# kessel/dune-pnp

Hardware: NVIDIA B200
Metric: newton_step_dofs_per_s (higher is better)
Workload: dtype f64

## Files before the change

### dune_pnp_b200/csrc/pnp_amg.cu

```cuda
#include <cub/cub.cuh>
#include <cusolverDn.h>

#include <chrono>
#include <cmath>
#include <cstdlib>
#include <cstring>

#include "pnp_common.cuh"
#include "pnp_spmv_tma.cuh"
#include "pnp_sweep.cuh"

namespace pnp {

std::shared_ptr<SweepPlan> sweep_plan_build(Ctx&, const SweepView&, int F);
void sweep_gs(Ctx&, const SweepPlan&, const SweepView&, const double* vals, long stride, const double* d, double* x, int dir);

namespace {

constexpr int BLK = 256;

struct Level {
  int nv = 0; long nslots = 0;
  const int* rp = nullptr; const unsigned* col = nullptr; const double* vals = nullptr;
  DBuf<int> rp_own; DBuf<unsigned> col_own; DBuf<double> vals_own;
  DBuf<double> dinv, x, x2, b, r;
  double lmax = 2.0;
  DBuf<int> agg, par1;
  DBuf<int> agg_ptr, agg_mem;
  DBuf<int> seg_ptr, seg_items;
  DBuf<unsigned char> seg_w;
  double alpha = 1.0;
  Ctx* lc = nullptr;
  Vec u; Matrix Amat;
  const unsigned char* dm = nullptr;
  bool redisc = false;
  DBuf<XY> xy_own; DBuf<unsigned char> dmask_own;
  std::shared_ptr<SweepPlan> gs_plan;
};

}

struct Amg {
  int NP = 1, F = 1;
  bool symbolic = false;
  long nv0 = -1, nslots0 = -1;
  long mg_epoch = -1;
  double sym_key = 0.0;
  double omega = 0.7, alpha = 1.6;
  int coarse_sweeps = 40;
  int gamma = 1;
  int wlevels = 99;
  int smoother = 0;
  double cheb_ratio = 8.0;
  int comp0 = 0;
  int pre_steps = -1, post_steps = -1;
  int dense_max = 4096, dense_n = 0;
  cusolverDnHandle_t cus = nullptr;
  DBuf<double> dense, dense_work;
  DBuf<int> dense_piv, dense_info;
  bool distributed = false;
  bool redisc = false;
  DBuf<double> grhs;
  std::unique_ptr<Solver> rep_solver; Matrix rep_A; Vec rep_u; DBuf<double> rep_x;
  int n_geo = 0;
  std::vector<std::unique_ptr<Level>> L;
  DBuf<unsigned char> tmp;
  void* temp(size_t bytes) { if (bytes > tmp.n) tmp.alloc(bytes); return tmp.p; }
  cudaGraphExec_t cg_exec = nullptr;
  bool cg_failed = false;
  int cg_calls = 0;
  double cg_key[8] = {0, 0, 0, 0, 0, 0, 0, 0};
  std::vector<std::pair<double*, double*>> cg_before, cg_after;
  long cg_launches = 0; double cg_bytes[Ctx::ACC_N] = {0, 0, 0, 0, 0, 0};
  void cg_reset() { if (cg_exec) cudaGraphExecDestroy(cg_exec); cg_exec = nullptr; cg_calls = 0; }
  ~Amg() { if (cg_exec) cudaGraphExecDestroy(cg_exec); if (cus) cusolverDnDestroy(cus); }
};

namespace {

__device__ __forceinline__ unsigned hash32(unsigned x) {
  x ^= x >> 16; x *= 0x7feb352du; x ^= x >> 15; x *= 0x846ca68bu; x ^= x >> 16;
  return x;
}
__global__ void k_mis_select(const int* __restrict__ rp, const unsigned* __restrict__ col, int nv,
                             const unsigned char* __restrict__ st, unsigned char* __restrict__ st_out) {
  for (int v = blockIdx.x * blockDim.x + threadIdx.x; v < nv; v += gridDim.x * blockDim.x) {
    unsigned char s = st[v];
    if (s == 0) {
      const unsigned pv = hash32((unsigned)v);
      bool win = true;
      for (int k = rp[v] + 1; k < rp[v + 1]; k++) {
        const int w = (int)(col[k] & STAR_VMASK);
        if (w >= nv || w == v || st[w] != 0) continue;
        const unsigned pw = hash32((unsigned)w);
        if (pw > pv || (pw == pv && w > v)) { win = false; break; }
      }
      if (win) s = 1;
    }
    st_out[v] = s;
  }
}
__global__ void k_mis_cover(const int* __restrict__ rp, const unsigned* __restrict__ col, int nv,
                            unsigned char* __restrict__ st, int* __restrict__ undecided) {
  int local = 0;
  for (int v = blockIdx.x * blockDim.x + threadIdx.x; v < nv; v += gridDim.x * blockDim.x) {
    if (st[v] != 0) continue;
    bool covered = false;
    for (int k = rp[v] + 1; k < rp[v + 1]; k++) {
      const int w = (int)(col[k] & STAR_VMASK);
      if (w < nv && st[w] == 1) { covered = true; break; }
    }
    if (covered) st[v] = 2; else local++;
  }
  if (local) atomicAdd(undecided, local);
}
__global__ void k_root_flag(const unsigned char* __restrict__ st, int nv, int* __restrict__ flag) {
  for (int v = blockIdx.x * blockDim.x + threadIdx.x; v < nv; v += gridDim.x * blockDim.x) flag[v] = st[v] == 1;
}
__global__ void k_attach(const int* __restrict__ rp, const unsigned* __restrict__ col, const double* __restrict__ vals,
                         int nv, const unsigned char* __restrict__ st, const int* __restrict__ root_id,
                         int* __restrict__ agg) {
  for (int v = blockIdx.x * blockDim.x + threadIdx.x; v < nv; v += gridDim.x * blockDim.x) {
    if (st[v] == 1) { agg[v] = root_id[v]; continue; }
    double best = -1.0; int bw = -1;
    for (int k = rp[v] + 1; k < rp[v + 1]; k++) {
      const int w = (int)(col[k] & STAR_VMASK);
      if (w >= nv || st[w] != 1) continue;
      const double s = fabs(vals[k]);
      if (s > best || (s == best && w < bw)) { best = s; bw = w; }
    }
    agg[v] = root_id[bw];
  }
}
__global__ void k_coarse_keys(const int* __restrict__ rp, const unsigned* __restrict__ col, int nv,
                              const int* __restrict__ agg, uint64_t* __restrict__ keys, int* __restrict__ slot_id) {
  for (int v = blockIdx.x * blockDim.x + threadIdx.x; v < nv; v += gridDim.x * blockDim.x) {
    const unsigned I = (unsigned)agg[v];
    for (int k = rp[v]; k < rp[v + 1]; k++) {
      const unsigned w = col[k] & STAR_VMASK;
      if (w >= (unsigned)nv) { keys[k] = ~0ull; slot_id[k] = k; continue; }
      const unsigned J = (unsigned)agg[w];
      keys[k] = ((uint64_t)I << 32) | (J == I ? 0u : J + 1u);
      slot_id[k] = k;
    }
  }
}
__global__ void k_coarse_cols(const uint64_t* __restrict__ ukeys, long n, unsigned* __restrict__ col) {
  for (long i = blockIdx.x * (long)blockDim.x + threadIdx.x; i < n; i += (long)gridDim.x * blockDim.x) {
    const unsigned lo = (unsigned)(ukeys[i] & 0xffffffffu);
    col[i] = lo == 0 ? (unsigned)(ukeys[i] >> 32) : lo - 1u;
  }
}
__global__ void k_row_starts(const uint64_t* __restrict__ ukeys, long n, int nc, int* __restrict__ rp) {
  for (int I = blockIdx.x * blockDim.x + threadIdx.x; I <= nc; I += gridDim.x * blockDim.x)
    rp[I] = (int)lower_bound_u64(ukeys, n, (uint64_t)(unsigned)I << 32);
}
__global__ void k_lower_bounds_i32(const int* __restrict__ sorted, int n, int m, int* __restrict__ out) {
  for (int I = blockIdx.x * blockDim.x + threadIdx.x; I <= m; I += gridDim.x * blockDim.x) {
    int lo = 0, hi = n;
    while (lo < hi) { int mid = (lo + hi) >> 1; if (sorted[mid] < I) lo = mid + 1; else hi = mid; }
    out[I] = lo;
  }
}
__global__ void k_iota(int* a, int n) {
  for (int i = blockIdx.x * blockDim.x + threadIdx.x; i < n; i += gridDim.x * blockDim.x) a[i] = i;
}

template <int NP>
__global__ void k_galerkin(const int* __restrict__ seg_ptr, const int* __restrict__ seg_items,
                           const unsigned char* __restrict__ seg_w, long nsc, const double* __restrict__ vf, long nsf, double* __restrict__ vc,
                           const unsigned char* __restrict__ dmask, const unsigned* __restrict__ colf, const int* __restrict__ rpf,
                           int comp0) {
  for (long cs = blockIdx.x * (long)blockDim.x + threadIdx.x; cs < nsc; cs += (long)gridDim.x * blockDim.x) {
    double acc[NP];
#pragma unroll
    for (int p = 0; p < NP; p++) acc[p] = 0.0;
    constexpr int U = 4;
    const int t1 = seg_ptr[cs + 1];
    for (int t0 = seg_ptr[cs]; t0 < t1; t0 += U) {
      int s[U]; double w[U]; double v[U][NP];
#pragma unroll
      for (int q = 0; q < U; q++) {
        const bool ok = t0 + q < t1;
        s[q] = ok ? seg_items[t0 + q] : -1;
        const unsigned char wc = (ok && seg_w) ? seg_w[t0 + q] : 0;
        w[q] = ok ? (wc == 0 ? 1.0 : (wc == 1 ? 0.5 : 0.25)) : 0.0;
      }
#pragma unroll
      for (int q = 0; q < U; q++)
#pragma unroll
        for (int p = 0; p < NP; p++) v[q][p] = s[q] >= 0 ? vf[p * nsf + s[q]] : 0.0;
      if (dmask) {
#pragma unroll
        for (int q = 0; q < U; q++) {
          if (s[q] < 0) continue;
          const unsigned wv = colf[s[q]] & STAR_VMASK;
          const unsigned m = dmask[wv];
          if (m && rpf[wv] == s[q]) {
            if (NP == 1) { if ((m >> comp0) & 1u) v[q][0] = 0.0; }
            else if (NP == PNP_COMPACT_PLANES) { if (m & 1u) v[q][0] = 0.0; }
            else {
              if (m & 1u) v[q][0] = 0.0;
              if (m & 2u) v[q][NP == 7 ? 4 : 0] = 0.0;
              if (m & 4u) v[q][NP == 7 ? 6 : 0] = 0.0;
            }
          }
        }
      }
#pragma unroll
      for (int q = 0; q < U; q++)
        if (s[q] >= 0) {
#pragma unroll
          for (int p = 0; p < NP; p++) acc[p] += w[q] * v[q][p];
        }
    }
#pragma unroll
    for (int p = 0; p < NP; p++) vc[p * nsc + cs] = acc[p];
  }
}
template <int NP>
__global__ void k_dinv(const int* __restrict__ rp, const double* __restrict__ vals, long stride, int nv,
                       double* __restrict__ dinv) {
  for (int v = blockIdx.x * blockDim.x + threadIdx.x; v < nv; v += gridDim.x * blockDim.x) {
    const int s = rp[v];
    if (NP == 1) { const double d = vals[s]; dinv[v] = d != 0.0 ? 1.0 / d : 0.0; }
    else {
      const PnpBlock B = pnp_block_at<NP>(vals, stride, s);
      const double a = B.a, b = B.b, c_ = B.c, d = B.d, e = B.e, f = B.f, g = B.g;
      const double det = a * e * g - b * d * g - c_ * e * f;
      double* o = dinv + 9l * v;
      const double scale = fabs(a * e * g) + fabs(b * d * g) + fabs(c_ * e * f);
      if (fabs(det) > 1e-12 * scale && scale > 0.0) {
        const double id = 1.0 / det;
        o[0] = e * g * id;   o[1] = -b * g * id;           o[2] = -c_ * e * id;
        o[3] = -d * g * id;  o[4] = (a * g - c_ * f) * id; o[5] = c_ * d * id;
        o[6] = -e * f * id;  o[7] = b * f * id;            o[8] = (a * e - b * d) * id;
      } else {
        for (int i = 0; i < 9; i++) o[i] = 0.0;
        o[0] = a != 0.0 ? 1.0 / a : 0.0; o[4] = e != 0.0 ? 1.0 / e : 0.0; o[8] = g != 0.0 ? 1.0 / g : 0.0;
      }
    }
  }
}
template <int F>
__global__ void k_jacobi0(const double* __restrict__ dinv, const double* __restrict__ b, double omega,
                          double* __restrict__ x, int nv, double* __restrict__ dvec) {
  for (int v = blockIdx.x * blockDim.x + threadIdx.x; v < nv; v += gridDim.x * blockDim.x) {
    if (F == 1) {
      const double z = omega * dinv[v] * b[v];
      x[v] = z; if (dvec) dvec[v] = z;
    } else {
      const double* B = dinv + 9l * v;
      const double r0 = b[3l * v], r1 = b[3l * v + 1], r2 = b[3l * v + 2];
#pragma unroll
      for (int k = 0; k < 3; k++) {
        const double z = omega * (B[3 * k] * r0 + B[3 * k + 1] * r1 + B[3 * k + 2] * r2);
        x[3l * v + k] = z; if (dvec) dvec[3l * v + k] = z;
      }
    }
  }
}
template <int NP>
__global__ void k_gershgorin(const int* __restrict__ rp, const double* __restrict__ vals, long stride, int nv,
                             unsigned long long* __restrict__ out) {
  double best = 0.0;
  for (int v = blockIdx.x * blockDim.x + threadIdx.x; v < nv; v += gridDim.x * blockDim.x) {
    const int s0 = rp[v], s1 = rp[v + 1];
    if (NP == 1) {
      double sum = 0.0;
      for (int s = s0; s < s1; s++) sum += fabs(vals[s]);
      const double d = fabs(vals[s0]);
      if (d > 0.0) best = fmax(best, sum / d);
    } else {
      double s0_ = 0.0, s1_ = 0.0, s2_ = 0.0;
      for (int s = s0; s < s1; s++) {
        const PnpBlock B = pnp_block_at<NP>(vals, stride, s);
        s0_ += fabs(B.a) + fabs(B.b) + fabs(B.c);
        s1_ += fabs(B.d) + fabs(B.e);
        s2_ += fabs(B.f) + fabs(B.g);
      }
      const PnpBlock D = pnp_block_at<NP>(vals, stride, s0);
      const double d0 = fabs(D.a), d1 = fabs(D.e), d2 = fabs(D.g);
      if (d0 > 0.0) best = fmax(best, s0_ / d0);
      if (d1 > 0.0) best = fmax(best, s1_ / d1);
      if (d2 > 0.0) best = fmax(best, s2_ / d2);
    }
  }
  for (int o = 16; o > 0; o >>= 1) best = fmax(best, __shfl_xor_sync(0xffffffffu, best, o));
  if ((threadIdx.x & 31) == 0) atomicMax(out, (unsigned long long)__double_as_longlong(best));
}
template <int F>
__global__ void k_restrict(const int* __restrict__ agg_ptr, const int* __restrict__ agg_mem, const int* __restrict__ par1,
                           int nc, const double* __restrict__ r, double* __restrict__ bc) {
  for (int I = blockIdx.x * blockDim.x + threadIdx.x; I < nc; I += gridDim.x * blockDim.x) {
    double acc[F];
#pragma unroll
    for (int k = 0; k < F; k++) acc[k] = 0.0;
    for (int t = agg_ptr[I]; t < agg_ptr[I + 1]; t++) {
      const long v = agg_mem[t];
      const double w = (par1 && par1[v] >= 0) ? 0.5 : 1.0;
#pragma unroll
      for (int k = 0; k < F; k++) acc[k] += w * r[F * v + k];
    }
#pragma unroll
    for (int k = 0; k < F; k++) bc[(long)F * I + k] = acc[k];
  }
}
template <int F>
__global__ void k_prolong(const int* __restrict__ agg, const int* __restrict__ par1, int nv, const double* __restrict__ xc,
                          double alpha, double* __restrict__ x, const unsigned char* __restrict__ dmask, int comp0) {
  for (int v = blockIdx.x * blockDim.x + threadIdx.x; v < nv; v += gridDim.x * blockDim.x) {
    const long I = agg[v];
    const long J = par1 ? par1[v] : -1;
    const unsigned m = dmask ? (F == 3 ? dmask[v] : (dmask[v] >> comp0) & 1u) : 0u;
#pragma unroll
    for (int k = 0; k < F; k++)
      if (!((m >> k) & 1u))
        x[(long)F * v + k] += alpha * (J >= 0 ? 0.5 * (xc[F * I + k] + xc[F * J + k]) : xc[F * I + k]);
  }
}
__global__ void k_level_geometry(const int* __restrict__ int2ext_c, const int* __restrict__ ext2int_f, const XY* __restrict__ xy_f,
                                 const unsigned char* __restrict__ dmask_f, int nvc, XY* __restrict__ xy_c,
                                 unsigned char* __restrict__ dmask_c) {
  for (int i = blockIdx.x * blockDim.x + threadIdx.x; i < nvc; i += gridDim.x * blockDim.x) {
    const int j = ext2int_f[int2ext_c[i]];
    xy_c[i] = xy_f[j]; dmask_c[i] = dmask_f[j];
  }
}
__global__ void k_geo_parents(const int* __restrict__ int2ext_f, int nvf, int nvc, const uint64_t* __restrict__ edges,
                              const int* __restrict__ ext2int_c, int* __restrict__ par0, int* __restrict__ par1) {
  for (int i = blockIdx.x * blockDim.x + threadIdx.x; i < nvf; i += gridDim.x * blockDim.x) {
    const int e = int2ext_f[i];
    if (e < nvc) { par0[i] = ext2int_c[e]; par1[i] = -1; }
    else {
      const uint64_t k = edges[e - nvc];
      par0[i] = ext2int_c[(int)(k >> 32)]; par1[i] = ext2int_c[(int)(k & 0xffffffffu)];
    }
  }
}
__global__ void k_geo_pairs(const int* __restrict__ par0, const int* __restrict__ par1, int nvf, int nrows_c,
                            int* __restrict__ key, int* __restrict__ val) {
  for (int i = blockIdx.x * blockDim.x + threadIdx.x; i < nvf; i += gridDim.x * blockDim.x) {
    key[2 * i] = (par0[i] >= 0 && par0[i] < nrows_c) ? par0[i] : 0x7fffffff; val[2 * i] = i;
    key[2 * i + 1] = (par1[i] >= 0 && par1[i] < nrows_c) ? par1[i] : 0x7fffffff; val[2 * i + 1] = i;
  }
}
template <int F>
__global__ void k_inject(const int* __restrict__ par0, const int* __restrict__ par1, int nvf, const double* __restrict__ uf,
                         double* __restrict__ uc) {
  for (int i = blockIdx.x * blockDim.x + threadIdx.x; i < nvf; i += gridDim.x * blockDim.x)
    if (par1[i] < 0 && par0[i] >= 0) {
#pragma unroll
      for (int k = 0; k < F; k++) uc[(long)F * par0[i] + k] = uf[(long)F * i + k];
    }
}
template <int F>
__global__ void k_mask_dirichlet(double* __restrict__ b, const unsigned char* __restrict__ dmask, int nv, int comp0) {
  for (int v = blockIdx.x * blockDim.x + threadIdx.x; v < nv; v += gridDim.x * blockDim.x) {
    const unsigned m = F == 3 ? dmask[v] : (dmask[v] >> comp0) & 1u;
#pragma unroll
    for (int k = 0; k < F; k++) if ((m >> k) & 1u) b[(long)F * v + k] = 0.0;
  }
}
template <int NP>
__global__ void k_dense_fill_global(const int* __restrict__ rp, const unsigned* __restrict__ col, const double* __restrict__ vals,
                                    long stride, int nrows, const int* __restrict__ gid, double* __restrict__ Ad, long n,
                                    const unsigned char* __restrict__ dmask, int comp0) {
  constexpr int F = NP == 1 ? 1 : 3;
  for (int r = blockIdx.x * blockDim.x + threadIdx.x; r < nrows; r += gridDim.x * blockDim.x) {
    const long rg = gid[r];
    for (int s = rp[r]; s < rp[r + 1]; s++) {
      const long cg = gid[col[s] & STAR_VMASK];
      const unsigned dm = (dmask && s == rp[r]) ? dmask[r] : 0u;
      if (NP == 1) { if (!((dm >> comp0) & 1u)) atomicAdd(&Ad[cg * n + rg], vals[s]); }
      else {
        const PnpBlock B = pnp_block_at<NP>(vals, stride, s);
#pragma unroll
        for (int ki = 0; ki < 3; ki++)
#pragma unroll
          for (int kj = 0; kj < 3; kj++)
            if (pnp_plane(ki, kj) >= 0 && !(ki == kj && ((dm >> ki) & 1u))) atomicAdd(&Ad[(F * cg + kj) * n + F * rg + ki], B.at(ki, kj));
      }
    }
  }
}
template <int F>
__global__ void k_to_global(const double* __restrict__ loc, const int* __restrict__ gid, int nrows, double* __restrict__ glob) {
  for (int v = blockIdx.x * blockDim.x + threadIdx.x; v < nrows; v += gridDim.x * blockDim.x)
#pragma unroll
    for (int k = 0; k < F; k++) atomicAdd(&glob[(long)F * gid[v] + k], loc[(long)F * v + k]);
}
template <int F>
__global__ void k_add_from_global(const double* __restrict__ glob, const int* __restrict__ gid, int nrows, double alpha,
                                  double* __restrict__ x, const unsigned char* __restrict__ dmask, int comp0) {
  for (int v = blockIdx.x * blockDim.x + threadIdx.x; v < nrows; v += gridDim.x * blockDim.x) {
    const unsigned m = F == 3 ? dmask[v] : (dmask[v] >> comp0) & 1u;
#pragma unroll
    for (int k = 0; k < F; k++) if (!((m >> k) & 1u)) x[(long)F * v + k] += alpha * glob[(long)F * gid[v] + k];
  }
}
template <int F>
__global__ void k_from_global(const double* __restrict__ glob, const int* __restrict__ gid, int nloc, double* __restrict__ loc) {
  for (int v = blockIdx.x * blockDim.x + threadIdx.x; v < nloc; v += gridDim.x * blockDim.x)
#pragma unroll
    for (int k = 0; k < F; k++) loc[(long)F * v + k] = glob[(long)F * gid[v] + k];
}
__device__ __forceinline__ int find_slot(const int* rp, const unsigned* col, int I, int J) {
  for (int s = rp[I]; s < rp[I + 1]; s++) if ((int)(col[s] & STAR_VMASK) == J) return s;
  return -1;
}
__global__ void k_geo_items(const int* __restrict__ rpf, const unsigned* __restrict__ colf, int nvf,
                            const int* __restrict__ par0, const int* __restrict__ par1, const int* __restrict__ rpc,
                            const unsigned* __restrict__ colc, int* __restrict__ key, unsigned* __restrict__ val,
                            int* __restrict__ err) {
  for (int i = blockIdx.x * blockDim.x + threadIdx.x; i < nvf; i += gridDim.x * blockDim.x) {
    const int I[2] = {par0[i], par1[i]};
    for (int s = rpf[i]; s < rpf[i + 1]; s++) {
      const int j = (int)(colf[s] & STAR_VMASK);
      const int J[2] = {par0[j], par1[j]};
#pragma unroll
      for (int a = 0; a < 2; a++)
#pragma unroll
        for (int b = 0; b < 2; b++) {
          const long o = 4l * s + 2 * a + b;
          if (I[a] < 0 || J[b] < 0) { key[o] = 0x7fffffff; val[o] = 0; continue; }
          const int cs = find_slot(rpc, colc, I[a], J[b]);
          if (cs < 0) { atomicExch(err, 1); key[o] = 0x7fffffff; val[o] = 0; continue; }
          const unsigned wc = (I[1] >= 0 ? 1u : 0u) + (J[1] >= 0 ? 1u : 0u);
          key[o] = cs; val[o] = (unsigned)s | (wc << 29);
        }
    }
  }
}
__global__ void k_geo_unpack(const unsigned* __restrict__ val, long n, int* __restrict__ items, unsigned char* __restrict__ w) {
  for (long t = blockIdx.x * (long)blockDim.x + threadIdx.x; t < n; t += (long)gridDim.x * blockDim.x) {
    items[t] = (int)(val[t] & 0x1fffffffu); w[t] = (unsigned char)(val[t] >> 29);
  }
}

#define KL(c, kern, n, ...)                                                                              \
  do { kern<<<grid_for((n), BLK), BLK, 0, (c).stream>>>(__VA_ARGS__); PNP_CHECK_LAUNCH(); (c).launches++; } while (0)

template <int EPI>
void level_op(Ctx& c, const Amg& A, const Level& l, const double* x, const double* b, double* y, double omega_or_c2 = -1.0,
              double c1 = 0.0, double* dvec = nullptr) {
  StarOpArgs a{l.rp, l.col, l.vals, l.nslots, l.nv, x, y};
  a.b = b; a.dinv = l.dinv.p; a.block = A.F == 3; a.omega = omega_or_c2 < 0 ? A.omega : omega_or_c2; a.c1 = c1; a.dvec = dvec;
  const bool fine = &l == A.L[0].get();
  if (A.distributed) halo_exchange(*l.lc, const_cast<double*>(x), A.F);
  if (fine) c.prof_mark(EPI == EPI_RESIDUAL ? 1 : 2);
  launch_star_op_auto<EPI, 0>(c, A.NP, a, fine);
  if (fine) c.prof_mark();
}

bool coarsen(Ctx& c, Amg& A, int li) {
  Level& f = *A.L[li];
  const int nv = f.nv;
  DBuf<unsigned char> st(nv), st2(nv);
  st.zero(c.stream);
  DBuf<int> d_und(1);
  for (int round = 0; round < 200; round++) {
    KL(c, k_mis_select, nv, f.rp, f.col, nv, st.p, st2.p);
    std::swap(st.p, st2.p);
    d_und.zero(c.stream);
    KL(c, k_mis_cover, nv, f.rp, f.col, nv, st.p, d_und.p);
    int und = 0;
    d_und.download(&und, 1, c.stream);
    if (und == 0) break;
    PNP_REQUIRE(round < 199, PNP_E_ARG, "AMG: independent-set selection did not terminate");
  }
  DBuf<int> flag(nv), root_id(nv);
  KL(c, k_root_flag, nv, st.p, nv, flag.p);
  size_t bytes = 0;
  cub::DeviceScan::ExclusiveSum(nullptr, bytes, flag.p, root_id.p, nv, c.stream);
  PNP_CUDA(cub::DeviceScan::ExclusiveSum(A.temp(bytes), bytes, flag.p, root_id.p, nv, c.stream));
  int last_id = 0, last_flag = 0;
  PNP_CUDA(cudaMemcpyAsync(&last_id, root_id.p + nv - 1, sizeof(int), cudaMemcpyDeviceToHost, c.stream));
  PNP_CUDA(cudaMemcpyAsync(&last_flag, flag.p + nv - 1, sizeof(int), cudaMemcpyDeviceToHost, c.stream));
  PNP_CUDA(cudaStreamSynchronize(c.stream));
  const int nc = last_id + last_flag;
  if (nc < 1 || nc > 0.8 * nv) return false;
  f.alpha = A.alpha;
  f.agg.alloc(nv);
  KL(c, k_attach, nv, f.rp, f.col, f.vals, nv, st.p, root_id.p, f.agg.p);
  {
    DBuf<int> ids(nv), agg_sorted(nv);
    f.agg_mem.alloc(nv); f.agg_ptr.alloc(nc + 1);
    KL(c, k_iota, nv, ids.p, nv);
    cub::DeviceRadixSort::SortPairs(nullptr, bytes, f.agg.p, agg_sorted.p, ids.p, f.agg_mem.p, nv, 0, 32, c.stream);
    PNP_CUDA(cub::DeviceRadixSort::SortPairs(A.temp(bytes), bytes, f.agg.p, agg_sorted.p, ids.p, f.agg_mem.p, nv, 0, 32,
                                            c.stream));
    KL(c, k_lower_bounds_i32, nc + 1, agg_sorted.p, nv, nc, f.agg_ptr.p);
  }
  auto nl = std::make_unique<Level>();
  {
    const long ns = f.nslots;
    PNP_REQUIRE(ns < (1l << 31), PNP_E_MESH, "AMG: too many matrix slots on one level");
    DBuf<uint64_t> keys(ns), skeys(ns), ukeys(ns);
    DBuf<int> slot(ns), counts(ns + 1), d_nu(1);
    f.seg_items.alloc(ns);
    KL(c, k_coarse_keys, nv, f.rp, f.col, nv, f.agg.p, keys.p, slot.p);
    cub::DeviceRadixSort::SortPairs(nullptr, bytes, keys.p, skeys.p, slot.p, f.seg_items.p, (int)ns, 0, 64, c.stream);
    PNP_CUDA(cub::DeviceRadixSort::SortPairs(A.temp(bytes), bytes, keys.p, skeys.p, slot.p, f.seg_items.p, (int)ns, 0, 64,
                                            c.stream));
    cub::DeviceRunLengthEncode::Encode(nullptr, bytes, skeys.p, ukeys.p, counts.p, d_nu.p, (int)ns, c.stream);
    PNP_CUDA(cub::DeviceRunLengthEncode::Encode(A.temp(bytes), bytes, skeys.p, ukeys.p, counts.p, d_nu.p, (int)ns, c.stream));
    int nu = 0;
    d_nu.download(&nu, 1, c.stream);
    {
      uint64_t lastkey = 0;
      PNP_CUDA(cudaMemcpyAsync(&lastkey, ukeys.p + (nu - 1), sizeof(uint64_t), cudaMemcpyDeviceToHost, c.stream));
      PNP_CUDA(cudaStreamSynchronize(c.stream));
      if (lastkey == ~0ull) nu--;
    }
    nl->nv = nc; nl->nslots = nu;
    PNP_CUDA(cudaMemsetAsync(counts.p + nu, 0, sizeof(int), c.stream));
    f.seg_ptr.alloc((size_t)nu + 1);
    cub::DeviceScan::ExclusiveSum(nullptr, bytes, counts.p, f.seg_ptr.p, nu + 1, c.stream);
    PNP_CUDA(cub::DeviceScan::ExclusiveSum(A.temp(bytes), bytes, counts.p, f.seg_ptr.p, nu + 1, c.stream));
    nl->rp_own.alloc((size_t)nc + 1); nl->col_own.alloc(nu);
    KL(c, k_row_starts, nc + 1, ukeys.p, (long)nu, nc, nl->rp_own.p);
    KL(c, k_coarse_cols, nu, ukeys.p, (long)nu, nl->col_own.p);
    c.launches += 8;
    PNP_CUDA(cudaStreamSynchronize(c.stream));
  }
  nl->vals_own.alloc((size_t)A.NP * nl->nslots);
  nl->rp = nl->rp_own.p; nl->col = nl->col_own.p; nl->vals = nl->vals_own.p;
  A.L.push_back(std::move(nl));
  return true;
}

void coarsen_geometric(Ctx& c, Amg& A, int li, const HierLevel& h, const int* int2ext_f, bool redisc) {
  Level& f = *A.L[li];
  const int nvf = f.nv, nvc = (int)h.nv;
  size_t bytes = 0;
  f.agg.alloc(nvf); f.par1.alloc(nvf);
  KL(c, k_geo_parents, nvf, int2ext_f, nvf, nvc, h.edges.p, h.ext2int.p, f.agg.p, f.par1.p);
  {
    DBuf<int> key(2 * (size_t)nvf), val(2 * (size_t)nvf), skey(2 * (size_t)nvf), sval(2 * (size_t)nvf);
    KL(c, k_geo_pairs, nvf, f.agg.p, f.par1.p, nvf, nvc, key.p, val.p);
    cub::DeviceRadixSort::SortPairs(nullptr, bytes, key.p, skey.p, val.p, sval.p, 2 * nvf, 0, 32, c.stream);
    PNP_CUDA(cub::DeviceRadixSort::SortPairs(A.temp(bytes), bytes, key.p, skey.p, val.p, sval.p, 2 * nvf, 0, 32, c.stream));
    f.agg_ptr.alloc((size_t)nvc + 1);
    KL(c, k_lower_bounds_i32, nvc + 1, skey.p, 2 * nvf, nvc, f.agg_ptr.p);
    int nvalid = 0;
    PNP_CUDA(cudaMemcpyAsync(&nvalid, f.agg_ptr.p + nvc, sizeof(int), cudaMemcpyDeviceToHost, c.stream));
    PNP_CUDA(cudaStreamSynchronize(c.stream));
    f.agg_mem.alloc(nvalid);
    PNP_CUDA(cudaMemcpyAsync(f.agg_mem.p, sval.p, (size_t)nvalid * sizeof(int), cudaMemcpyDeviceToDevice, c.stream));
    PNP_CUDA(cudaStreamSynchronize(c.stream));
  }
  auto nl = std::make_unique<Level>();
  nl->nv = nvc; nl->nslots = h.nslots; nl->rp = h.rp.p; nl->col = h.adj.p;
  nl->redisc = redisc;
  if (redisc) {
    nl->xy_own.alloc(nvc); nl->dmask_own.alloc(nvc);
    KL(c, k_level_geometry, nvc, h.int2ext.p, c.ext2int.p, c.xy.p, c.dmask.p, nvc, nl->xy_own.p, nl->dmask_own.p);
    nl->dm = nl->dmask_own.p;
    nl->u.fields = A.F; nl->u.d.alloc((size_t)A.F * nvc);
  } else {
    const long n4 = 4 * f.nslots;
    PNP_REQUIRE(n4 < (1l << 31) && f.nslots < (1l << 29), PNP_E_MESH, "multigrid: too many matrix slots on one level");
    DBuf<int> key(n4), skey(n4), err(1);
    DBuf<unsigned> val(n4), sval(n4);
    err.zero(c.stream);
    KL(c, k_geo_items, nvf, f.rp, f.col, nvf, f.agg.p, f.par1.p, nl->rp, nl->col, key.p, val.p, err.p);
    int herr = 0;
    err.download(&herr, 1, c.stream);
    PNP_REQUIRE(herr == 0, PNP_E_MESH, "multigrid: refinement levels are not nested");
    cub::DeviceRadixSort::SortPairs(nullptr, bytes, key.p, skey.p, val.p, sval.p, (int)n4, 0, 32, c.stream);
    PNP_CUDA(cub::DeviceRadixSort::SortPairs(A.temp(bytes), bytes, key.p, skey.p, val.p, sval.p, (int)n4, 0, 32, c.stream));
    key.release(); val.release();
    f.seg_ptr.alloc((size_t)nl->nslots + 1);
    KL(c, k_lower_bounds_i32, nl->nslots + 1, skey.p, (int)n4, (int)nl->nslots, f.seg_ptr.p);
    int nvalid = 0;
    PNP_CUDA(cudaMemcpyAsync(&nvalid, f.seg_ptr.p + nl->nslots, sizeof(int), cudaMemcpyDeviceToHost, c.stream));
    PNP_CUDA(cudaStreamSynchronize(c.stream));
    f.seg_items.alloc(nvalid); f.seg_w.alloc(nvalid);
    KL(c, k_geo_unpack, nvalid, sval.p, (long)nvalid, f.seg_items.p, f.seg_w.p);
    PNP_CUDA(cudaStreamSynchronize(c.stream));
    c.launches += 4;
  }
  f.alpha = 1.0;
  nl->vals_own.alloc((size_t)A.NP * nl->nslots);
  nl->vals = nl->vals_own.p;
  A.L.push_back(std::move(nl));
}

void alloc_work(Ctx& c, Amg& A, Level& l) {
  const size_t n = (size_t)A.F * l.nv, nall = (A.distributed && l.lc) ? (size_t)A.F * l.lc->nv : n;
  l.dinv.alloc(A.F == 3 ? 9 * (size_t)l.nv : n); l.x.alloc(nall); l.x2.alloc(nall); l.b.alloc(nall); l.r.alloc(nall);
  l.x.zero(c.stream); l.x2.zero(c.stream); l.b.zero(c.stream); l.r.zero(c.stream);
}

void coarsen_distributed(Ctx& c, Amg& A, int li, MgLevelRef& ref) {
  Level& f = *A.L[li];
  Ctx& fc = *f.lc; Ctx& kc = *ref.lc;
  const int nvf_all = (int)fc.nv, nvc = (int)kc.n_own;
  size_t bytes = 0;
  f.agg.alloc(nvf_all); f.par1.alloc(nvf_all);
  PNP_CUDA(cudaMemcpyAsync(f.agg.p, ref.par0.p, nvf_all * sizeof(int), cudaMemcpyDeviceToDevice, c.stream));
  PNP_CUDA(cudaMemcpyAsync(f.par1.p, ref.par1.p, nvf_all * sizeof(int), cudaMemcpyDeviceToDevice, c.stream));
  {
    DBuf<int> key(2 * (size_t)nvf_all), val(2 * (size_t)nvf_all), skey(2 * (size_t)nvf_all), sval(2 * (size_t)nvf_all);
    KL(c, k_geo_pairs, nvf_all, f.agg.p, f.par1.p, nvf_all, nvc, key.p, val.p);
    cub::DeviceRadixSort::SortPairs(nullptr, bytes, key.p, skey.p, val.p, sval.p, 2 * nvf_all, 0, 32, c.stream);
    PNP_CUDA(cub::DeviceRadixSort::SortPairs(A.temp(bytes), bytes, key.p, skey.p, val.p, sval.p, 2 * nvf_all, 0, 32, c.stream));
    f.agg_ptr.alloc((size_t)nvc + 1);
    KL(c, k_lower_bounds_i32, nvc + 1, skey.p, 2 * nvf_all, nvc, f.agg_ptr.p);
    int nvalid = 0;
    PNP_CUDA(cudaMemcpyAsync(&nvalid, f.agg_ptr.p + nvc, sizeof(int), cudaMemcpyDeviceToHost, c.stream));
    PNP_CUDA(cudaStreamSynchronize(c.stream));
    f.agg_mem.alloc(nvalid);
    PNP_CUDA(cudaMemcpyAsync(f.agg_mem.p, sval.p, (size_t)nvalid * sizeof(int), cudaMemcpyDeviceToDevice, c.stream));
    PNP_CUDA(cudaStreamSynchronize(c.stream));
  }
  f.alpha = 1.0;
  auto nl = std::make_unique<Level>();
  nl->lc = &kc; nl->nv = nvc; nl->nslots = kc.nslots; nl->rp = kc.rp.p; nl->col = kc.adj.p;
  nl->dm = kc.dmask.p;
  nl->u.fields = A.F; nl->u.d.alloc((size_t)A.F * kc.nv); nl->u.d.zero(c.stream);
  nl->Amat.op = A.F == 3 ? OP_PNP : OP_PB; nl->Amat.nplanes = A.NP;
  nl->Amat.vals.alloc((size_t)A.NP * kc.nslots);
  nl->vals = nl->Amat.vals.p;
  A.L.push_back(std::move(nl));
}

void dense_factor(Ctx& c, Amg& A);

void dense_factor_global(Ctx& c, Amg& A);
void replica_setup(Ctx& c, Amg& A);

const double* level_values(Ctx& c, Amg& A, int li, const double* uf, int comp0) {
  Level& l = *A.L[li]; Level& n = *A.L[li + 1];
  if (n.redisc) {
    if (A.F == 1) KL(c, k_inject<1>, l.nv, l.agg.p, l.par1.p, l.nv, uf, n.u.d.p);
    else KL(c, k_inject<3>, l.nv, l.agg.p, l.par1.p, l.nv, uf, n.u.d.p);
    c.acct(Ctx::ACC_TRANSFER, 8.0 * l.nv + 16.0 * A.F * n.nv);
    Operator op = c.last_op; op.aux0 = op.aux1 = -1;
    assemble_jacobian_on(c, StarView{n.rp, n.col, n.xy_own.p, n.dmask_own.p, n.nv}, n.nslots, op, n.u.d.p, n.vals_own.p,
                         A.NP, c.last_mode, c.last_eps);
    return n.u.d.p;
  }
  if (A.NP == 1)
    KL(c, k_galerkin<1>, n.nslots, l.seg_ptr.p, l.seg_items.p, l.seg_w.p, n.nslots, l.vals, l.nslots, n.vals_own.p, l.dm, l.col, l.rp, comp0);
  else if (A.NP == PNP_COMPACT_PLANES)
    KL(c, k_galerkin<PNP_COMPACT_PLANES>, n.nslots, l.seg_ptr.p, l.seg_items.p, l.seg_w.p, n.nslots, l.vals, l.nslots, n.vals_own.p, l.dm, l.col, l.rp, comp0);
  else
    KL(c, k_galerkin<7>, n.nslots, l.seg_ptr.p, l.seg_items.p, l.seg_w.p, n.nslots, l.vals, l.nslots, n.vals_own.p, l.dm, l.col, l.rp, comp0);
  c.acct(Ctx::ACC_ASSEMBLY, 8.0 * A.NP * ((double)l.nslots + (double)n.nslots) + 5.0 * (double)l.seg_items.n + 4.0 * (double)n.nslots);
  return nullptr;
}

void level_dinv(Ctx& c, Amg& A, Level& l) {
  if (A.NP == 1) KL(c, k_dinv<1>, l.nv, l.rp, l.vals, l.nslots, l.nv, l.dinv.p);
  else if (A.NP == PNP_COMPACT_PLANES) KL(c, k_dinv<PNP_COMPACT_PLANES>, l.nv, l.rp, l.vals, l.nslots, l.nv, l.dinv.p);
  else KL(c, k_dinv<7>, l.nv, l.rp, l.vals, l.nslots, l.nv, l.dinv.p);
}

void gershgorin_bounds(Ctx& c, Amg& A) {
  DBuf<unsigned long long> d_l(A.L.size());
  d_l.zero(c.stream);
  for (size_t li = 0; li < A.L.size(); li++) {
    Level& l = *A.L[li];
    if (A.NP == 1) KL(c, k_gershgorin<1>, l.nv, l.rp, l.vals, l.nslots, l.nv, d_l.p + li);
    else if (A.NP == PNP_COMPACT_PLANES) KL(c, k_gershgorin<PNP_COMPACT_PLANES>, l.nv, l.rp, l.vals, l.nslots, l.nv, d_l.p + li);
    else KL(c, k_gershgorin<7>, l.nv, l.rp, l.vals, l.nslots, l.nv, d_l.p + li);
  }
  if (A.distributed) allreduce_max_u64(c, d_l.p, A.L.size());
  std::vector<unsigned long long> h = d_l.to_host(c.stream);
  for (size_t li = 0; li < A.L.size(); li++) {
    double v; std::memcpy(&v, &h[li], sizeof v);
    A.L[li]->lmax = (v > 0.0 && std::isfinite(v)) ? v : 2.0;
  }
}

void numeric(Ctx& c, Amg& A, int comp0) {
  if (A.distributed) {
    PNP_REQUIRE(c.last_u, PNP_E_ARG, "distributed multigrid needs the state of the last Jacobian assembly (the vector must stay alive)");
    PNP_REQUIRE(c.last_vals == A.L[0]->vals, PNP_E_ARG,
                "distributed multigrid re-discretises its coarse levels: the matrix must be the Jacobian of the last assembly");
    const double* uf = c.last_u;
    for (size_t li = 0; li + 1 < A.L.size(); li++) {
      Level& l = *A.L[li]; Level& n = *A.L[li + 1];
      const int nvf_all = (int)l.lc->nv;
      if (A.F == 1) KL(c, k_inject<1>, nvf_all, l.agg.p, l.par1.p, nvf_all, uf, n.u.d.p);
      else KL(c, k_inject<3>, nvf_all, l.agg.p, l.par1.p, nvf_all, uf, n.u.d.p);
      c.acct(Ctx::ACC_TRANSFER, 8.0 * nvf_all + 16.0 * A.F * n.nv);
      Operator op = c.last_op; op.aux0 = op.aux1 = -1;
      n.Amat.op = op.op;
      n.lc->launches = 0;
      assemble_jacobian(*n.lc, op, n.u, n.Amat, c.last_mode, c.last_eps);
      c.absorb(*n.lc);
      uf = n.u.d.p;
    }
    for (size_t li = 0; li < A.L.size(); li++) {
      Level& l = *A.L[li];
      level_dinv(c, A, l);
      c.acct(Ctx::ACC_ASSEMBLY, (4.0 + 8.0 * A.NP + (A.F == 3 ? 72.0 : 8.0)) * l.nv);
    }
    if (c.mg_replica) replica_setup(c, A); else dense_factor_global(c, A);
    if (A.smoother == 1) gershgorin_bounds(c, A);
    return;
  }
  const double* uf = c.last_u;
  for (size_t li = 0; li < A.L.size(); li++) {
    Level& l = *A.L[li];
    if (li + 1 < A.L.size()) uf = level_values(c, A, (int)li, uf, comp0);
    level_dinv(c, A, l);
    c.acct(Ctx::ACC_ASSEMBLY, (4.0 + 8.0 * A.NP + (A.F == 3 ? 72.0 : 8.0)) * l.nv);
  }
  A.dense_n = 0;
  if ((long)A.F * A.L.back()->nv <= A.dense_max) dense_factor(c, A);
  if (A.smoother == 1) gershgorin_bounds(c, A);
}

template <int NP>
__global__ void k_dense_fill(const int* __restrict__ rp, const unsigned* __restrict__ col, const double* __restrict__ vals,
                             long stride, int nv, double* __restrict__ Ad, long n) {
  constexpr int F = NP == 1 ? 1 : 3;
  for (int r = blockIdx.x * blockDim.x + threadIdx.x; r < nv; r += gridDim.x * blockDim.x)
    for (int s = rp[r]; s < rp[r + 1]; s++) {
      const long cidx = col[s] & STAR_VMASK;
      if (cidx >= nv) continue;
      if (NP == 1) Ad[cidx * n + r] = vals[s];
      else {
        const PnpBlock B = pnp_block_at<NP>(vals, stride, s);
#pragma unroll
        for (int ki = 0; ki < 3; ki++)
#pragma unroll
          for (int kj = 0; kj < 3; kj++)
            if (pnp_plane(ki, kj) >= 0) Ad[(F * cidx + kj) * n + F * r + ki] = B.at(ki, kj);
      }
    }
}
__global__ void k_dense_fix_diag(double* __restrict__ Ad, long n) {
  for (long i = blockIdx.x * (long)blockDim.x + threadIdx.x; i < n; i += (long)gridDim.x * blockDim.x)
    if (Ad[i * n + i] == 0.0) Ad[i * n + i] = 1.0;
}
#define PNP_CUSOLVER(call)                                                                                          \
  do { cusolverStatus_t s_ = (call); if (s_ != CUSOLVER_STATUS_SUCCESS)                                             \
    throw ::pnp::Error(PNP_E_CUDA, std::string(#call) + " -> cusolver status " + std::to_string((int)s_)); } while (0)

void dense_factor(Ctx& c, Amg& A) {
  Level& l = *A.L.back();
  const long n = (long)A.F * l.nv;
  A.dense_n = (int)n;
  if (!A.cus) PNP_CUSOLVER(cusolverDnCreate(&A.cus));
  PNP_CUSOLVER(cusolverDnSetStream(A.cus, c.stream));
  if (A.dense.n != (size_t)(n * n)) { A.dense.alloc(n * n); A.dense_piv.alloc(n); A.dense_info.alloc(1); }
  A.dense.zero(c.stream);
  if (A.NP == 1) KL(c, k_dense_fill<1>, l.nv, l.rp, l.col, l.vals, l.nslots, l.nv, A.dense.p, n);
  else if (A.NP == PNP_COMPACT_PLANES) KL(c, k_dense_fill<PNP_COMPACT_PLANES>, l.nv, l.rp, l.col, l.vals, l.nslots, l.nv, A.dense.p, n);
  else KL(c, k_dense_fill<7>, l.nv, l.rp, l.col, l.vals, l.nslots, l.nv, A.dense.p, n);
  KL(c, k_dense_fix_diag, n, A.dense.p, n);
  int lwork = 0;
  PNP_CUSOLVER(cusolverDnDgetrf_bufferSize(A.cus, (int)n, (int)n, A.dense.p, (int)n, &lwork));
  if (A.dense_work.n < (size_t)lwork) A.dense_work.alloc(lwork);
  PNP_CUSOLVER(cusolverDnDgetrf(A.cus, (int)n, (int)n, A.dense.p, (int)n, A.dense_work.p, A.dense_piv.p, A.dense_info.p));
  c.acct(Ctx::ACC_DENSE, 24.0 * (double)n * (double)n);
  int info = 0;
  A.dense_info.download(&info, 1, c.stream);
  PNP_REQUIRE(info == 0, PNP_E_BREAKDOWN, "multigrid: coarsest-level matrix is singular (LU info " + std::to_string(info) + ")");
}
void dense_solve(Ctx& c, Amg& A, Level& l) {
  const long n = A.dense_n;
  PNP_CUDA(cudaMemcpyAsync(l.x.p, l.b.p, n * sizeof(double), cudaMemcpyDeviceToDevice, c.stream));
  PNP_CUSOLVER(cusolverDnDgetrs(A.cus, CUBLAS_OP_N, (int)n, 1, A.dense.p, (int)n, A.dense_piv.p, l.x.p, (int)n, A.dense_info.p));
  c.launches += 2; c.acct(Ctx::ACC_DENSE, 8.0 * (double)n * (double)n);
}

void dense_factor_global(Ctx& c, Amg& A) {
  Level& l = *A.L.back();
  const long n = (long)A.F * c.mg_nglobal;
  A.dense_n = (int)n;
  if (!A.cus) PNP_CUSOLVER(cusolverDnCreate(&A.cus));
  PNP_CUSOLVER(cusolverDnSetStream(A.cus, c.stream));
  if (A.dense.n != (size_t)(n * n)) { A.dense.alloc(n * n); A.dense_piv.alloc(n); A.dense_info.alloc(1); A.grhs.alloc(n); }
  A.dense.zero(c.stream);
  const unsigned char* dm = c.mg_aggregated ? l.lc->dmask.p : nullptr;
  if (A.NP == 1) KL(c, k_dense_fill_global<1>, l.nv, l.rp, l.col, l.vals, l.nslots, l.nv, c.mg_gid.p, A.dense.p, n, dm, A.comp0);
  else if (A.NP == PNP_COMPACT_PLANES)
    KL(c, k_dense_fill_global<PNP_COMPACT_PLANES>, l.nv, l.rp, l.col, l.vals, l.nslots, l.nv, c.mg_gid.p, A.dense.p, n, dm, A.comp0);
  else KL(c, k_dense_fill_global<7>, l.nv, l.rp, l.col, l.vals, l.nslots, l.nv, c.mg_gid.p, A.dense.p, n, dm, A.comp0);
  allreduce_sum(c, A.dense.p, (size_t)(n * n));
  KL(c, k_dense_fix_diag, n, A.dense.p, n);
  int lwork = 0;
  PNP_CUSOLVER(cusolverDnDgetrf_bufferSize(A.cus, (int)n, (int)n, A.dense.p, (int)n, &lwork));
  if (A.dense_work.n < (size_t)lwork) A.dense_work.alloc(lwork);
  static const bool timing = std::getenv("PNP_AMG_TIMING") != nullptr;
  if (timing) PNP_CUDA(cudaStreamSynchronize(c.stream));
  const auto t0 = std::chrono::steady_clock::now();
  PNP_CUSOLVER(cusolverDnDgetrf(A.cus, (int)n, (int)n, A.dense.p, (int)n, A.dense_work.p, A.dense_piv.p, A.dense_info.p));
  int info = 0;
  A.dense_info.download(&info, 1, c.stream);
  if (timing) std::printf("[amg] rank %d global dense LU n = %ld: %.1f ms\n", c.rank, n,
                          1e3 * std::chrono::duration<double>(std::chrono::steady_clock::now() - t0).count());
  PNP_REQUIRE(info == 0, PNP_E_BREAKDOWN, "multigrid: coarsest-level matrix is singular (LU info " + std::to_string(info) + ")");
}
void dense_correct_aggregated(Ctx& c, Amg& A, Level& l) {
  const long n = A.dense_n;
  A.grhs.zero(c.stream);
  if (A.F == 1) KL(c, k_to_global<1>, l.nv, l.r.p, c.mg_gid.p, l.nv, A.grhs.p);
  else KL(c, k_to_global<3>, l.nv, l.r.p, c.mg_gid.p, l.nv, A.grhs.p);
  allreduce_sum(c, A.grhs.p, (size_t)n);
  PNP_CUSOLVER(cusolverDnDgetrs(A.cus, CUBLAS_OP_N, (int)n, 1, A.dense.p, (int)n, A.dense_piv.p, A.grhs.p, (int)n, A.dense_info.p));
  if (A.F == 1) KL(c, k_add_from_global<1>, l.nv, A.grhs.p, c.mg_gid.p, l.nv, A.alpha, l.x.p, l.lc->dmask.p, A.comp0);
  else KL(c, k_add_from_global<3>, l.nv, A.grhs.p, c.mg_gid.p, l.nv, A.alpha, l.x.p, l.lc->dmask.p, A.comp0);
  c.launches += 2;
}
void dense_solve_global(Ctx& c, Amg& A, Level& l) {
  const long n = A.dense_n;
  A.grhs.zero(c.stream);
  if (A.F == 1) KL(c, k_to_global<1>, l.nv, l.b.p, c.mg_gid.p, l.nv, A.grhs.p);
  else KL(c, k_to_global<3>, l.nv, l.b.p, c.mg_gid.p, l.nv, A.grhs.p);
  allreduce_sum(c, A.grhs.p, (size_t)n);
  PNP_CUSOLVER(cusolverDnDgetrs(A.cus, CUBLAS_OP_N, (int)n, 1, A.dense.p, (int)n, A.dense_piv.p, A.grhs.p, (int)n, A.dense_info.p));
  const int nloc = (int)l.lc->nv;
  if (A.F == 1) KL(c, k_from_global<1>, nloc, A.grhs.p, c.mg_gid.p, nloc, l.x.p);
  else KL(c, k_from_global<3>, nloc, A.grhs.p, c.mg_gid.p, nloc, l.x.p);
  c.launches += 2;
}

}
void amg_setup(Ctx& c, Solver& S, const Matrix& M);
void amg_apply(Ctx& c, Solver& S, const Matrix&, const double* d, double* y);
namespace {
void replica_setup(Ctx& c, Amg& A) {
  Ctx& rc = *c.mg_replica;
  Level& l = *A.L.back();
  const long n = (long)A.F * c.mg_nglobal;
  A.dense_n = (int)n;
  if (A.grhs.n != (size_t)n) { A.grhs.alloc(n); A.rep_x.alloc(n); A.rep_u.d.alloc(n); }
  A.rep_u.fields = A.F;
  A.rep_u.d.zero(c.stream);
  if (A.F == 1) KL(c, k_to_global<1>, l.nv, l.u.d.p, c.mg_gid.p, l.nv, A.rep_u.d.p);
  else KL(c, k_to_global<3>, l.nv, l.u.d.p, c.mg_gid.p, l.nv, A.rep_u.d.p);
  allreduce_sum(c, A.rep_u.d.p, (size_t)n);
  Operator op = c.last_op; op.aux0 = op.aux1 = -1;
  A.rep_A.op = op.op; A.rep_A.nplanes = A.NP;
  if (A.rep_A.vals.n != (size_t)A.NP * rc.nslots) A.rep_A.vals.alloc((size_t)A.NP * rc.nslots);
  rc.launches = 0;
  assemble_jacobian(rc, op, A.rep_u, A.rep_A, c.last_mode, c.last_eps);
  if (!A.rep_solver) { A.rep_solver = std::make_unique<Solver>(); A.rep_solver->prec = PNP_PREC_AMG; }
  auto& ro = A.rep_solver->opts;
  ro["amg_geometric"] = 1;  ro["amg_omega"] = A.omega; ro["amg_alpha"] = A.alpha; ro["amg_gamma"] = A.gamma;
  ro["amg_dense_max"] = A.dense_max; ro["amg_coarse_sweeps"] = A.coarse_sweeps; ro["amg_smoother"] = A.smoother;
  ro["amg_cheb_ratio"] = A.cheb_ratio; ro["amg_pre_steps"] = A.pre_steps; ro["amg_post_steps"] = A.post_steps;
  amg_setup(rc, *A.rep_solver, A.rep_A);
  c.absorb(rc);
}
void replica_solve(Ctx& c, Amg& A, Level& l, int nu) {
  Ctx& rc = *c.mg_replica;
  const long n = (long)A.F * c.mg_nglobal;
  A.grhs.zero(c.stream);
  if (A.F == 1) KL(c, k_to_global<1>, l.nv, l.b.p, c.mg_gid.p, l.nv, A.grhs.p);
  else KL(c, k_to_global<3>, l.nv, l.b.p, c.mg_gid.p, l.nv, A.grhs.p);
  allreduce_sum(c, A.grhs.p, (size_t)n);
  A.rep_solver->prec_steps = nu;
  rc.launches = 0;
  amg_apply(rc, *A.rep_solver, A.rep_A, A.grhs.p, A.rep_x.p);
  const int nloc = (int)l.lc->nv;
  if (A.F == 1) KL(c, k_from_global<1>, nloc, A.rep_x.p, c.mg_gid.p, nloc, l.x.p);
  else KL(c, k_from_global<3>, nloc, A.rep_x.p, c.mg_gid.p, nloc, l.x.p);
  c.absorb(rc); c.launches += 2;
}

void jacobi0(Ctx& c, Amg& A, Level& l, double omega, double* dvec) {
  if (A.F == 1) KL(c, k_jacobi0<1>, l.nv, l.dinv.p, l.b.p, omega, l.x.p, l.nv, dvec);
  else KL(c, k_jacobi0<3>, l.nv, l.dinv.p, l.b.p, omega, l.x.p, l.nv, dvec);
  c.acct(Ctx::ACC_TRANSFER, ((A.F == 3 ? 72.0 : 8.0) + 16.0 * A.F + (dvec ? 8.0 * A.F : 0.0)) * l.nv);
}

void smooth(Ctx& c, Amg& A, Level& l, int steps, bool zero) {
  const long n = (long)A.F * l.nv;
  if (steps <= 0) { if (zero) PNP_CUDA(cudaMemsetAsync(l.x.p, 0, n * sizeof(double), c.stream)); return; }
  if (A.smoother == 0) {
    int s = 0;
    if (zero) { jacobi0(c, A, l, A.omega, nullptr); s = 1; }
    for (; s < steps; s++) { level_op<2>(c, A, l, l.x.p, l.b.p, l.x2.p); std::swap(l.x.p, l.x2.p); }
    return;
  }
  if (A.smoother == 2) {
    const bool finest = &l == A.L[0].get();
    const SweepView V{l.rp, l.col, finest ? c.int2ext.p : nullptr, l.nv};
    if (!l.gs_plan) l.gs_plan = sweep_plan_build(c, V, A.F);
    if (zero) PNP_CUDA(cudaMemsetAsync(l.x.p, 0, n * sizeof(double), c.stream));
    for (int s = 0; s < steps; s++) {
      sweep_gs(c, *l.gs_plan, V, l.vals, l.nslots, l.b.p, l.x.p, +1);
      sweep_gs(c, *l.gs_plan, V, l.vals, l.nslots, l.b.p, l.x.p, -1);
    }
    c.acct(finest ? Ctx::ACC_SPMV_FINE : Ctx::ACC_SPMV_COARSE, 2.0 * steps * ((8.0 * A.NP + 4.0) * (double)l.nslots + 24.0 * n));
    return;
  }
  const double lmx = 1.1 * l.lmax, lmn = l.lmax / A.cheb_ratio;
  const double theta = 0.5 * (lmx + lmn), delta = 0.5 * (lmx - lmn), sigma = theta / delta;
  double rho = 1.0 / sigma;
  int s = 0;
  if (zero) { jacobi0(c, A, l, 1.0 / theta, l.r.p); s = 1; }
  else { level_op<3>(c, A, l, l.x.p, l.b.p, l.x2.p, 1.0 / theta, 0.0, l.r.p); std::swap(l.x.p, l.x2.p); s = 1; }
  for (; s < steps; s++) {
    const double rho_new = 1.0 / (2.0 * sigma - rho);
    level_op<3>(c, A, l, l.x.p, l.b.p, l.x2.p, 2.0 * rho_new / delta, rho_new * rho, l.r.p);
    std::swap(l.x.p, l.x2.p);
    rho = rho_new;
  }
}

void cycle(Ctx& c, Amg& A, int li, int nu, int comp0, bool zero);

void coarse_correction(Ctx& c, Amg& A, int nu, int comp0) {
  auto direct = [&] {
    const int visits = 0 < A.wlevels ? A.gamma : 1;
    for (int g = 0; g < visits; g++) cycle(c, A, 1, nu, comp0, g == 0);
  };
  auto snapshot = [&](std::vector<std::pair<double*, double*>>& v) {
    v.clear();
    for (size_t li = 1; li < A.L.size(); li++) v.push_back({A.L[li]->x.p, A.L[li]->x2.p});
  };
  auto restore = [&](const std::vector<std::pair<double*, double*>>& v) {
    for (size_t li = 1; li < A.L.size(); li++) { A.L[li]->x.p = v[li - 1].first; A.L[li]->x2.p = v[li - 1].second; }
  };
  cudaStreamCaptureStatus cap = cudaStreamCaptureStatusNone;
  PNP_CUDA(cudaStreamIsCapturing(c.stream, &cap));
  if (!tune().graph || A.cg_failed || A.smoother != 0 || cap != cudaStreamCaptureStatusNone) { direct(); return; }
  const double key[8] = {(double)nu, A.omega, (double)A.gamma, (double)A.wlevels, (double)A.pre_steps, (double)A.post_steps,
                         (double)A.coarse_sweeps, (double)comp0 + 16.0 * A.dense_n};
  if (A.cg_exec && std::memcmp(key, A.cg_key, sizeof key) != 0) A.cg_reset();
  if (!A.cg_exec) {
    if (A.cg_calls++ < 1) { direct(); return; }
    std::memcpy(A.cg_key, key, sizeof key);
    snapshot(A.cg_before);
    const long l0 = c.launches;
    double b0[Ctx::ACC_N];
    for (int k = 0; k < Ctx::ACC_N; k++) b0[k] = c.alg_bytes[k];
    cudaGraph_t graph = nullptr;
    bool ok = cudaStreamBeginCapture(c.stream, cudaStreamCaptureModeThreadLocal) == cudaSuccess;
    if (ok) {
      try { direct(); } catch (const Error&) { ok = false; }
      if (cudaStreamEndCapture(c.stream, &graph) != cudaSuccess || !graph) ok = false;
    }
    if (ok && cudaGraphInstantiate(&A.cg_exec, graph, 0) != cudaSuccess) { ok = false; A.cg_exec = nullptr; }
    if (graph) cudaGraphDestroy(graph);
    A.cg_launches = c.launches - l0; c.launches = l0;
    for (int k = 0; k < Ctx::ACC_N; k++) { A.cg_bytes[k] = c.alg_bytes[k] - b0[k]; c.alg_bytes[k] = b0[k]; }
    snapshot(A.cg_after);
    if (!ok) {
      cudaGetLastError();
      A.cg_failed = true; A.cg_exec = nullptr;
      restore(A.cg_before);
      direct();
      return;
    }
  }
  restore(A.cg_before);
  PNP_CUDA(cudaGraphLaunch(A.cg_exec, c.stream));
  restore(A.cg_after);
  c.launches += A.cg_launches;
  for (int k = 0; k < Ctx::ACC_N; k++) c.alg_bytes[k] += A.cg_bytes[k];
}

void cycle(Ctx& c, Amg& A, int li, int nu, int comp0, bool zero) {
  Level& l = *A.L[li];
  const bool coarsest = li + 1 == (int)A.L.size();
  if (coarsest && A.dense_n > 0 && A.distributed && c.mg_aggregated) {
    smooth(c, A, l, nu, zero);
    level_op<1>(c, A, l, l.x.p, l.b.p, l.r.p);
    dense_correct_aggregated(c, A, l);
    smooth(c, A, l, nu, false);
    return;
  }
  if (coarsest && A.dense_n > 0) {
    if (A.distributed && c.mg_replica) replica_solve(c, A, l, nu);
    else if (A.distributed) dense_solve_global(c, A, l);
    else dense_solve(c, A, l);
    return;
  }
  const int nu_pre = A.pre_steps >= 0 ? A.pre_steps : nu, nu_post = A.post_steps >= 0 ? A.post_steps : nu;
  smooth(c, A, l, coarsest ? A.coarse_sweeps : nu_pre, zero);
  if (coarsest) return;
  Level& nx = *A.L[li + 1];
  level_op<1>(c, A, l, l.x.p, l.b.p, l.r.p);
  if (A.distributed) halo_exchange(*l.lc, l.r.p, A.F);
  if (A.F == 1) KL(c, k_restrict<1>, nx.nv, l.agg_ptr.p, l.agg_mem.p, l.par1.p, nx.nv, l.r.p, nx.b.p);
  else KL(c, k_restrict<3>, nx.nv, l.agg_ptr.p, l.agg_mem.p, l.par1.p, nx.nv, l.r.p, nx.b.p);
  c.acct(Ctx::ACC_TRANSFER, (8.0 * A.F + 4.0) * l.nv + 4.0 * (double)l.agg_mem.n + (8.0 * A.F + 4.0) * nx.nv);
  if (nx.dm) {
    if (A.F == 1) KL(c, k_mask_dirichlet<1>, nx.nv, nx.b.p, nx.dm, nx.nv, comp0);
    else KL(c, k_mask_dirichlet<3>, nx.nv, nx.b.p, nx.dm, nx.nv, comp0);
    c.acct(Ctx::ACC_TRANSFER, 1.0 * nx.nv);
  }
  if (li == 0) coarse_correction(c, A, nu, comp0);
  else {
    const int visits = li < A.wlevels ? A.gamma : 1;
    for (int g = 0; g < visits; g++) cycle(c, A, li + 1, nu, comp0, g == 0);
  }
  if (A.distributed && !(li + 2 == (int)A.L.size() && A.dense_n > 0 && !c.mg_aggregated)) halo_exchange(*nx.lc, nx.x.p, A.F);
  const unsigned char* dm = l.dm;
  if (A.F == 1) KL(c, k_prolong<1>, l.nv, l.agg.p, l.par1.p, l.nv, nx.x.p, l.alpha, l.x.p, dm, comp0);
  else KL(c, k_prolong<3>, l.nv, l.agg.p, l.par1.p, l.nv, nx.x.p, l.alpha, l.x.p, dm, comp0);
  c.acct(Ctx::ACC_TRANSFER, (16.0 * A.F + 9.0) * l.nv + 8.0 * A.F * nx.nv);
  smooth(c, A, l, nu_post, false);
}

}

int amg_graph_state(const Solver& S) { return !S.amg ? 0 : (S.amg->cg_exec ? 1 : (S.amg->cg_failed ? -1 : 0)); }

void amg_setup(Ctx& c, Solver& S, const Matrix& M) {
  if (!S.amg) S.amg = std::make_shared<Amg>();
  Amg& A = *S.amg;
  const int comp0 = M.comp0;
  A.comp0 = comp0;
  const bool want_redisc = S.opt("amg_geometric", 1) != 0 && S.opt("amg_rediscretise", 1) != 0 && c.n_own == c.nv &&
                           !c.hier.empty() && c.mg.empty() && c.last_u && c.last_vals == M.vals.p &&
                           (M.op == OP_PB || M.op == OP_PNP || M.op == OP_MASS);
  const double sym_key = S.opt("amg_geometric", 1) + 3.0 * S.opt("amg_dense_max", 4096) + 1e7 * S.opt("amg_alpha", 1.6);
  if (!A.symbolic || A.NP != M.nplanes || A.nv0 != c.n_own || A.nslots0 != c.nslots || A.redisc != want_redisc ||
      A.mg_epoch != c.mg_epoch || A.sym_key != sym_key) {
    A.L.clear(); A.cg_reset(); A.cg_failed = false;
    A.NP = M.nplanes; A.F = M.nplanes == 1 ? 1 : 3;
    A.nv0 = c.n_own; A.nslots0 = c.nslots; A.mg_epoch = c.mg_epoch; A.sym_key = sym_key;
    auto l0 = std::make_unique<Level>();
    l0->nv = (int)c.n_own; l0->nslots = c.nslots; l0->rp = c.rp.p; l0->col = c.adj.p; l0->vals = M.vals.p;
    A.L.push_back(std::move(l0));
    A.alpha = S.opt("amg_alpha", 1.6);
    A.L[0]->lc = &c;
    A.L[0]->dm = c.dmask.p;
    A.redisc = want_redisc;
    A.distributed = S.opt("amg_geometric", 1) != 0 && !c.mg.empty() && c.mg_nglobal > 0 &&
                    (M.op == OP_PB || M.op == OP_PNP || M.op == OP_MASS);
    if (A.distributed) {
      for (auto& ref : c.mg) coarsen_distributed(c, A, (int)A.L.size() - 1, ref);
      A.n_geo = (int)c.mg.size();
    }
    const bool geometric = !A.distributed && S.opt("amg_geometric", 1) != 0 && c.n_own == c.nv && !c.hier.empty();
    if (!A.distributed) A.n_geo = 0;
    if (geometric) {
      const int* i2e = c.int2ext.p;
      const double* uf = c.last_u;
      for (int hi = (int)c.hier.size() - 1; hi >= 0; hi--) {
        const int li = (int)A.L.size() - 1;
        coarsen_geometric(c, A, li, c.hier[hi], i2e, A.redisc);
        i2e = c.hier[hi].int2ext.p;
        uf = level_values(c, A, li, uf, comp0);
        A.n_geo++;
      }
    }
    A.dense_max = (int)S.opt("amg_dense_max", 4096);
    for (int li = (int)A.L.size() - 1; li < 24 && !A.distributed; li++) {
      if (A.L[li]->nv <= 64 || (long)A.F * A.L[li]->nv <= A.dense_max) break;
      if (!coarsen(c, A, li)) break;
      level_values(c, A, li, nullptr, comp0);
    }
    for (auto& l : A.L) alloc_work(c, A, *l);
    if (!A.distributed) {
      Level& l0r = *A.L[0];
      const size_t nall = (size_t)A.F * c.nv;
      l0r.x.alloc(nall); l0r.x2.alloc(nall);
      l0r.x.zero(c.stream); l0r.x2.zero(c.stream);
    }
    A.symbolic = true;
    if (S.verbosity > 0) {
      std::printf("multigrid hierarchy (%d geometric transfers):", A.n_geo);
      for (auto& l : A.L) std::printf(" %d", l->nv);
      std::printf("\n");
    }
  }
  A.L[0]->vals = M.vals.p;
  static const bool timing = std::getenv("PNP_AMG_TIMING") != nullptr;
  if (timing) PNP_CUDA(cudaStreamSynchronize(c.stream));
  const auto t_num0 = std::chrono::steady_clock::now();
  A.omega = S.opt("amg_omega", 0.7); A.gamma = (int)S.opt("amg_gamma", 1); A.wlevels = (int)S.opt("amg_wlevels", 99);
  A.coarse_sweeps = (int)S.opt("amg_coarse_sweeps", 40); A.smoother = (int)S.opt("amg_smoother", 0);
  PNP_REQUIRE(A.smoother >= 0 && A.smoother <= 2, PNP_E_ARG, "amg_smoother: 0 damped Jacobi, 1 Chebyshev, 2 symmetric Gauss-Seidel");
  PNP_REQUIRE(A.smoother != 2 || !A.distributed, PNP_E_ARG, "the Gauss-Seidel smoother sweeps the rows of one GPU: use Jacobi / Chebyshev on a partitioned mesh");
  PNP_REQUIRE(A.smoother != 2 || A.NP != PNP_COMPACT_PLANES, PNP_E_ARG, "the Gauss-Seidel smoother sweeps 7-plane PNP matrices only");
  A.cheb_ratio = S.opt("amg_cheb_ratio", 8.0);
  A.pre_steps = (int)S.opt("amg_pre_steps", -1); A.post_steps = (int)S.opt("amg_post_steps", -1);
  numeric(c, A, comp0);
  if (timing) {
    PNP_CUDA(cudaStreamSynchronize(c.stream));
    std::printf("[amg] rank %d numeric setup %.1f ms (levels %zu, dense n = %d, distributed %d)\n", c.rank,
                1e3 * std::chrono::duration<double>(std::chrono::steady_clock::now() - t_num0).count(), A.L.size(), A.dense_n,
                (int)A.distributed);
  }
}

void amg_apply(Ctx& c, Solver& S, const Matrix&, const double* d, double* y) {
  Amg& A = *S.amg;
  Level& l0 = *A.L[0];
  const long n = (long)A.F * l0.nv;
  const int nu = S.prec_steps > 0 ? S.prec_steps : 1;
  if (c.n_own == c.nv) {
    double *keep_b = l0.b.p, *keep_x = l0.x.p, *keep_x2 = l0.x2.p;
    const int pre = A.pre_steps >= 0 ? A.pre_steps : nu, post = A.post_steps >= 0 ? A.post_steps : nu;
    const int swaps = A.smoother == 2 ? 0 : (pre > 0 ? pre - 1 : 0) + post;
    struct Restore {
      Level& l; double *b, *x, *x2;
      ~Restore() { l.b.p = b; l.x.p = x; l.x2.p = x2; }
    } restore{l0, keep_b, keep_x, keep_x2};
    l0.b.p = const_cast<double*>(d);
    if (swaps & 1) l0.x2.p = y; else l0.x.p = y;
    cycle(c, A, 0, nu, A.comp0, true);
    double* result = l0.x.p;
    if (result != y) { PNP_CUDA(cudaMemcpyAsync(y, result, n * sizeof(double), cudaMemcpyDeviceToDevice, c.stream)); c.acct(Ctx::ACC_BLAS1, 16.0 * n); }
    return;
  }
  PNP_CUDA(cudaMemcpyAsync(l0.b.p, d, n * sizeof(double), cudaMemcpyDeviceToDevice, c.stream));
  cycle(c, A, 0, nu, A.comp0, true);
  PNP_CUDA(cudaMemcpyAsync(y, l0.x.p, n * sizeof(double), cudaMemcpyDeviceToDevice, c.stream));
}

}
```

### dune_pnp_b200/csrc/pnp_capi.cu

```cuda
#include <cuda_profiler_api.h>

#include <cstring>

#include "pnp_common.cuh"

namespace pnp {
int newton_apply(Ctx&, const Operator&, Vec&, Solver&, const pnp_newton_opts&, pnp_newton_result&);
int amg_graph_state(const Solver&);
LinResult slp_apply(Ctx&, const Operator&, Vec&, Solver&, double, int, double);
int onestep_apply(Ctx&, int, const Operator&, const Operator&, Solver&, double, Vec&, Vec&, Vec&, double, int, double, LinResult*);
namespace {
__global__ void k_fill(double* x, long n, double v) {
  for (long i = blockIdx.x * (long)blockDim.x + threadIdx.x; i < n; i += (long)gridDim.x * blockDim.x) x[i] = v;
}
__global__ void k_pack3(const double* a, const double* b, const double* c, long nv, double* out) {
  for (long i = blockIdx.x * (long)blockDim.x + threadIdx.x; i < nv; i += (long)gridDim.x * blockDim.x) {
    out[3 * i] = a[i]; out[3 * i + 1] = b[i]; out[3 * i + 2] = c[i];
  }
}
__global__ void k_extract(const double* in, long nv, int field, double* out) {
  for (long i = blockIdx.x * (long)blockDim.x + threadIdx.x; i < nv; i += (long)gridDim.x * blockDim.x) out[i] = in[3 * i + field];
}
void to_lin(const LinResult& lr, pnp_lin_result* out) {
  if (!out) return;
  out->converged = lr.converged; out->iterations = lr.iterations; out->reduction = lr.reduction;
  out->conv_rate = lr.conv_rate; out->seconds = lr.seconds; out->status = lr.status;
}
}
}

using namespace pnp;


#define API_BEGIN(ctx)                                  \
  if (!(ctx)) return PNP_E_ARG;                         \
  Ctx& c = (ctx)->c;                                    \
  try {                                                 \
    PNP_CUDA(cudaSetDevice(c.device));
#define API_END                                                      \
    return PNP_OK;                                                   \
  } catch (const pnp::Error& e) { c.err = e.what(); return e.code; } \
  catch (const std::exception& e) { c.err = e.what(); return PNP_E_ARG; }

namespace pnp {
Ctx* ctx_make_owned_child(Ctx& p) {
  pnp_ctx* h = new pnp_ctx;
  h->c.device = p.device; h->c.stream = p.stream; h->c.owns_stream = false; h->c.sm_count = p.sm_count;
  h->c.params = p.params;
  h->c.parent = &p; p.children.push_back(&h->c);
  p.owned_children.push_back(h);
  return &h->c;
}
void ctx_destroy_owned_child(Ctx& p, Ctx* child) {
  for (size_t i = 0; i < p.owned_children.size(); i++) {
    pnp_ctx* h = (pnp_ctx*)p.owned_children[i];
    if (&h->c != child) continue;
    p.owned_children.erase(p.owned_children.begin() + i);
    pnp_ctx_destroy(h);
    return;
  }
}
}

extern "C" {

pnp_status pnp_ctx_create(int device, pnp_ctx** out) {
  if (!out) return PNP_E_ARG;
  *out = nullptr;
  int ndev = 0;
  if (cudaGetDeviceCount(&ndev) != cudaSuccess || device < 0 || device >= ndev) return PNP_E_CUDA;
  pnp_ctx* h = new pnp_ctx;
  h->c.device = device;
  if (cudaSetDevice(device) != cudaSuccess || cudaStreamCreate(&h->c.stream) != cudaSuccess) { delete h; return PNP_E_CUDA; }
  cudaDeviceGetAttribute(&h->c.sm_count, cudaDevAttrMultiProcessorCount, device);
  *out = h;
  return PNP_OK;
}
pnp_status pnp_ctx_create_child(pnp_ctx* parent, pnp_ctx** out) {
  if (!parent || !out) return PNP_E_ARG;
  pnp_ctx* h = new pnp_ctx;
  Ctx& p = parent->c;
  h->c.device = p.device; h->c.stream = p.stream; h->c.owns_stream = false; h->c.sm_count = p.sm_count;
  h->c.rank = p.rank; h->c.world = p.world; h->c.nccl = p.nccl;
  h->c.params = p.params;
  h->c.parent = &p; p.children.push_back(&h->c);
  *out = h;
  return PNP_OK;
}
void pnp_ctx_destroy(pnp_ctx* ctx) {
  if (!ctx) return;
  Ctx& c = ctx->c;
  cudaSetDevice(c.device);
  if (c.parent) {
    Ctx& p = *c.parent;
    for (size_t i = 0; i < p.children.size(); i++) if (p.children[i] == &c) { p.children.erase(p.children.begin() + i); break; }
    for (size_t i = 0; i < p.mg.size(); i++) if (p.mg[i].lc == &c) { p.mg.resize(i); p.mg_gid.release(); p.mg_nglobal = 0; p.mg_replica = nullptr; break; }
    if (p.mg_replica == &c) { p.mg_replica = nullptr; p.mg_gid.release(); p.mg_nglobal = 0; }
    p.mg_epoch++;
  }
  if (c.stream) cudaStreamSynchronize(c.stream);
  c.solvers.clear();
  {
    std::vector<void*> owned;
    owned.swap(c.owned_children);
    for (void* h : owned) pnp_ctx_destroy((pnp_ctx*)h);
  }
  for (Ctx* k : c.children) { k->solvers.clear(); k->parent = nullptr; k->stream = nullptr; k->nccl = nullptr; }
  if (c.h_red) cudaFreeHost(c.h_red);
  for (cudaEvent_t e : c.prof_ev) cudaEventDestroy(e);
  if (c.tm0) cudaEventDestroy(c.tm0);
  if (c.tm1) cudaEventDestroy(c.tm1);
  if (c.owns_comm) comm_destroy(c);
  cudaStream_t s = c.owns_stream ? c.stream : nullptr;
  delete ctx;
  if (s) cudaStreamDestroy(s);
}
pnp_status pnp_mg_push_level(pnp_ctx* ctx, pnp_ctx* child, const int* par0, const int* par1) {
  API_BEGIN(ctx)
  PNP_REQUIRE(c.degree == 1, PNP_E_ARG, "built for linear elements only");
  PNP_REQUIRE(child && par0 && par1, PNP_E_ARG, "null arguments");
  Ctx& f = c.mg.empty() ? c : *c.mg.back().lc;
  Ctx& k = child->c;
  PNP_REQUIRE(f.finalized && k.finalized, PNP_E_ARG, "both levels must be finalized");
  std::vector<int> fi2e = f.int2ext.to_host(c.stream), ke2i = k.ext2int.to_host(c.stream);
  std::vector<int> p0(f.nv), p1(f.nv);
  for (long i = 0; i < f.nv; i++) {
    const int e = fi2e[i];
    PNP_REQUIRE(par0[e] < k.nv && par1[e] < k.nv, PNP_E_ARG, "parent index out of range");
    p0[i] = par0[e] >= 0 ? ke2i[par0[e]] : -1;
    p1[i] = par1[e] >= 0 ? ke2i[par1[e]] : -1;
  }
  MgLevelRef r; r.lc = &k;
  r.par0.alloc(f.nv); r.par1.alloc(f.nv);
  r.par0.upload(p0.data(), f.nv, c.stream); r.par1.upload(p1.data(), f.nv, c.stream);
  PNP_CUDA(cudaStreamSynchronize(c.stream));
  c.mg.push_back(std::move(r));
  c.mg_epoch++;
  API_END
}
pnp_status pnp_mg_set_coarse_aggregates(pnp_ctx* ctx, const int* agg, long n_aggregates) {
  const pnp_status st = pnp_mg_set_coarse_global(ctx, agg, n_aggregates);
  if (st == PNP_OK) ctx->c.mg_aggregated = true;
  return st;
}
pnp_status pnp_mg_set_coarse_global(pnp_ctx* ctx, const int* gid, long n_global) {
  API_BEGIN(ctx)
  c.mg_aggregated = false; c.mg_replica = nullptr;
  PNP_REQUIRE(!c.mg.empty() && gid && n_global > 0, PNP_E_ARG, "no multigrid level pushed");
  Ctx& k = *c.mg.back().lc;
  std::vector<int> i2e = k.int2ext.to_host(c.stream), g(k.nv);
  for (long i = 0; i < k.nv; i++) { g[i] = gid[i2e[i]]; PNP_REQUIRE(g[i] >= 0 && g[i] < n_global, PNP_E_ARG, "global index out of range"); }
  c.mg_gid.alloc(k.nv); c.mg_gid.upload(g.data(), k.nv, c.stream);
  PNP_CUDA(cudaStreamSynchronize(c.stream));
  c.mg_nglobal = n_global; c.mg_epoch++;
  API_END
}
pnp_status pnp_mg_set_coarse_replica(pnp_ctx* ctx, pnp_ctx* replica, const int* gid, long n_global) {
  API_BEGIN(ctx)
  c.mg_aggregated = false; c.mg_replica = nullptr;
  PNP_REQUIRE(!c.mg.empty() && gid && n_global > 0 && replica, PNP_E_ARG, "no multigrid level pushed / null arguments");
  Ctx& k = *c.mg.back().lc;
  Ctx& r = replica->c;
  PNP_REQUIRE(r.finalized && r.n_own == r.nv && r.nv == n_global, PNP_E_ARG, "the replica must hold the whole coarsest mesh, finalized");
  std::vector<int> i2e = k.int2ext.to_host(c.stream), re2i = r.ext2int.to_host(c.stream), g(k.nv);
  for (long i = 0; i < k.nv; i++) {
    const int gi = gid[i2e[i]];
    PNP_REQUIRE(gi >= 0 && gi < n_global, PNP_E_ARG, "global index out of range");
    g[i] = re2i[gi];
  }
  c.mg_gid.alloc(k.nv); c.mg_gid.upload(g.data(), k.nv, c.stream);
  PNP_CUDA(cudaStreamSynchronize(c.stream));
  c.mg_nglobal = n_global; c.mg_replica = &r; c.mg_epoch++;
  API_END
}
pnp_status pnp_profile_spmv(pnp_ctx* ctx, int enable) {
  API_BEGIN(ctx) c.prof = enable != 0; c.prof_used = 0; API_END
}
pnp_status pnp_profile_spmv_get(pnp_ctx* ctx, long* launches, double* total_ms) {
  API_BEGIN(ctx)
  PNP_CUDA(cudaStreamSynchronize(c.stream));
  for (int k = 0; k < 3; k++) { if (launches) launches[k] = 0; if (total_ms) total_ms[k] = 0; }
  for (size_t i = 0; i + 1 < c.prof_used; i += 2) {
    float t = 0; PNP_CUDA(cudaEventElapsedTime(&t, c.prof_ev[i], c.prof_ev[i + 1]));
    const int k = c.prof_kind[i / 2];
    if (launches) launches[k]++;
    if (total_ms) total_ms[k] += t;
  }
  API_END
}
pnp_status pnp_profile_bytes(pnp_ctx* ctx, int reset, double* out6) {
  API_BEGIN(ctx)
  for (int k = 0; k < Ctx::ACC_N; k++) { if (out6) out6[k] = c.alg_bytes[k]; if (reset) c.alg_bytes[k] = 0; }
  API_END
}
pnp_status pnp_profiler_range(pnp_ctx* ctx, int start) {
  API_BEGIN(ctx)
  PNP_CUDA(cudaStreamSynchronize(c.stream));
  if (start) cudaProfilerStart(); else cudaProfilerStop();
  API_END
}
pnp_status pnp_timer_start(pnp_ctx* ctx) {
  API_BEGIN(ctx)
  if (!c.tm0) { PNP_CUDA(cudaEventCreate(&c.tm0)); PNP_CUDA(cudaEventCreate(&c.tm1)); }
  PNP_CUDA(cudaEventRecord(c.tm0, c.stream));
  API_END
}
pnp_status pnp_timer_stop(pnp_ctx* ctx, double* ms) {
  API_BEGIN(ctx)
  PNP_REQUIRE(c.tm0 && ms, PNP_E_ARG, "timer not started");
  PNP_CUDA(cudaEventRecord(c.tm1, c.stream));
  PNP_CUDA(cudaEventSynchronize(c.tm1));
  float t = 0; PNP_CUDA(cudaEventElapsedTime(&t, c.tm0, c.tm1));
  *ms = t;
  API_END
}
pnp_status pnp_tune(const char* name, double value) {
  if (!name) return PNP_E_ARG;
  const std::string n(name);
  Tune& t = tune();
  if (n == "tma") t.tma = value != 0;
  else if (n == "tma_stages") t.tma_stages = (int)value;
  else if (n == "tma_lpr") t.tma_lpr = (int)value;
  else if (n == "graph") t.graph = value != 0;
  else if (n == "fd_warp") t.fd_warp = value != 0;
  else if (n == "jac_compact") t.jac_compact = value != 0;
  else if (n == "p2_chunk") t.p2_chunk = (long)value;
  else if (n == "tma_min_rows") t.tma_min_rows = (long)value;
  else return PNP_E_ARG;
  return PNP_OK;
}
const char* pnp_last_error(pnp_ctx* ctx) { return ctx ? ctx->c.err.c_str() : "null context"; }
long pnp_launch_count(pnp_ctx* ctx) { return ctx ? ctx->c.launches : 0; }

pnp_status pnp_mesh_set(pnp_ctx* ctx, long nv, const double* x, const double* y, long nT, const int* tri, long nB,
                        const int* ba, const int* bb, const int* bphys) {
  API_BEGIN(ctx) mesh_set(c, nv, x, y, nT, tri, nB, ba, bb, bphys, nv); API_END
}
pnp_status pnp_mesh_set_local(pnp_ctx* ctx, long nv, long n_own, const double* x, const double* y, long nT, const int* tri,
                              long nB, const int* ba, const int* bb, const int* bphys) {
  API_BEGIN(ctx) mesh_set(c, nv, x, y, nT, tri, nB, ba, bb, bphys, n_own); API_END
}
pnp_status pnp_comm_unique_id(char* out128) {
  try { comm_unique_id(out128); return PNP_OK; } catch (...) { return PNP_E_CUDA; }
}
pnp_status pnp_comm_init(pnp_ctx* ctx, int rank, int world, const char* unique_id128) {
  API_BEGIN(ctx) comm_init(c, rank, world, unique_id128); API_END
}
pnp_status pnp_comm_init_file(pnp_ctx* ctx, int rank, int world, const char* path) {
  API_BEGIN(ctx)
  PNP_REQUIRE(world == 1 || path, PNP_E_ARG, "null rendezvous path");
  comm_bootstrap_file(c, rank, world, path ? path : "");
  API_END
}
pnp_status pnp_comm_allgatherv(pnp_ctx* ctx, const void* send, long nbytes, void* recv, long cap, long* counts) {
  API_BEGIN(ctx)
  PNP_REQUIRE(nbytes >= 0 && counts && (nbytes == 0 || send), PNP_E_ARG, "bad all-gather arguments");
  std::vector<long> cnt;
  std::vector<unsigned char> all = comm_allgatherv(c, send, nbytes, cnt);
  for (int r = 0; r < c.world; r++) counts[r] = cnt[r];
  if (recv) {
    PNP_REQUIRE((long)all.size() <= cap, PNP_E_ARG, "receive buffer too small");
    std::memcpy(recv, all.data(), all.size());
  }
  API_END
}
pnp_status pnp_halo_set(pnp_ctx* ctx, int n_nbr, const int* nbr, const int* send_ptr, const int* send_idx, const int* recv_ptr) {
  API_BEGIN(ctx) halo_set(c, n_nbr, nbr, send_ptr, send_idx, recv_ptr); API_END
}
pnp_status pnp_halo_exchange(pnp_ctx* ctx, int vec_handle) {
  API_BEGIN(ctx)
  PNP_REQUIRE(c.degree == 1, PNP_E_ARG, "built for linear elements only");
  halo_exchange(c, c.vec(vec_handle).d.p, c.vec(vec_handle).fields);
  PNP_CUDA(cudaStreamSynchronize(c.stream));
  API_END
}
pnp_status pnp_mesh_read_gmsh(pnp_ctx* ctx, const char* path) {
  API_BEGIN(ctx)
  std::vector<double> x, y; std::vector<int> tri, ba, bb, ph;
  read_gmsh_file(path, x, y, tri, ba, bb, ph);
  mesh_set(c, (long)x.size(), x.data(), y.data(), (long)tri.size() / 3, tri.data(), (long)ba.size(), ba.data(), bb.data(),
           ph.data(), (long)x.size());
  API_END
}
pnp_status pnp_mesh_refine(pnp_ctx* ctx, int levels) { API_BEGIN(ctx) mesh_refine(c, levels); API_END }
pnp_status pnp_carry_set(pnp_ctx* ctx, const int* vec_handles, int n) { API_BEGIN(ctx) PNP_REQUIRE(c.degree == 1, PNP_E_ARG, "built for linear elements only"); carry_set(c, vec_handles, n); API_END }
pnp_status pnp_carry_get(pnp_ctx* ctx, int index, int vec_handle) { API_BEGIN(ctx) PNP_REQUIRE(c.degree == 1, PNP_E_ARG, "built for linear elements only"); carry_get(c, index, c.vec(vec_handle)); API_END }
pnp_status pnp_carry_set_host(pnp_ctx* ctx, int fields, const double* host) {
  API_BEGIN(ctx)
  PNP_REQUIRE(c.degree == 1, PNP_E_ARG, "built for linear elements only");
  PNP_REQUIRE(c.nv > 0 && fields >= 1 && host, PNP_E_ARG, "no mesh / bad field count");
  Vec cf; cf.fields = fields; cf.d.alloc((size_t)fields * c.nv);
  cf.d.upload(host, (size_t)fields * c.nv, c.stream);
  PNP_CUDA(cudaStreamSynchronize(c.stream));
  c.carry.clear();
  c.carry.push_back(std::move(cf));
  API_END
}
pnp_status pnp_carry_get_host(pnp_ctx* ctx, int index, double* host) {
  API_BEGIN(ctx)
  PNP_REQUIRE(c.degree == 1, PNP_E_ARG, "built for linear elements only");
  PNP_REQUIRE(index >= 0 && index < (int)c.carry.size() && host, PNP_E_ARG, "no such carried field");
  c.carry[index].d.download(host, c.carry[index].d.n, c.stream);
  API_END
}
pnp_status pnp_mesh_finalize(pnp_ctx* ctx, int renumber) { API_BEGIN(ctx) mesh_finalize(c, renumber != 0); API_END }
pnp_status pnp_mesh_sizes(pnp_ctx* ctx, long* nv, long* nT, long* nB, long* nslots) {
  API_BEGIN(ctx)
  if (nv) *nv = c.nv;
  if (nT) *nT = c.nT; if (nB) *nB = c.nB; if (nslots) *nslots = c.finalized ? c.nslots : 0;
  API_END
}
pnp_status pnp_mesh_get(pnp_ctx* ctx, double* x, double* y, int* tri, int* ba, int* bb, int* bphys) {
  API_BEGIN(ctx)
  if (x) c.cx.download(x, c.nv, c.stream);
  if (y) c.cy.download(y, c.nv, c.stream);
  if (tri) c.ctri.download(tri, 3 * c.nT, c.stream);
  if (ba) c.cba.download(ba, c.nB, c.stream);
  if (bb) c.cbb.download(bb, c.nB, c.stream);
  if (bphys) c.cbphys.download(bphys, c.nB, c.stream);
  API_END
}

pnp_status pnp_params_set(pnp_ctx* ctx, const double* sys, const double* surf) {
  API_BEGIN(ctx)
  PNP_REQUIRE(sys && (sys[0] == 0 || surf), PNP_E_ARG, "null parameter arrays");
  HostParams p;
  p.n_surfaces = (int)sys[0]; p.cylindrical = sys[1] != 0; p.l_b = sys[2]; p.c0 = sys[3]; p.PI = sys[4];
  p.linearSolverIterations = (int)sys[5]; p.newtonReassembleThreshold = sys[6]; p.newtonReduction = sys[7];
  p.newtonMinLinearReduction = sys[8]; p.newtonMaxIterations = sys[9]; p.newtonLineSearchMaxIteration = sys[10];
  p.tau = sys[11]; p.nSteps = (int)sys[12]; p.outputFreq = (int)sys[13]; p.potentialUpdateFreq = (int)sys[14];
  p.verbosity = (int)sys[15];
  PNP_REQUIRE(p.n_surfaces >= 0, PNP_E_CONFIG, "n_surfaces must be non-negative");
  p.surfaces.assign(p.n_surfaces, HostSurface());
  for (int i = 0; i < p.n_surfaces; i++)
    for (int k = 0; k < 3; k++) {
      p.surfaces[i].btype[k] = (int)surf[9 * i + 3 * k];
      p.surfaces[i].flux[k] = surf[9 * i + 3 * k + 1];
      p.surfaces[i].dval[k] = surf[9 * i + 3 * k + 2];
    }
  p.set = true;
  c.params = p;
  c.constraints_built = false;
  if (c.finalized) constraints_build(c);
  API_END
}
pnp_status pnp_params_read(pnp_ctx* ctx, const char* cfg_path) {
  API_BEGIN(ctx)
  read_config_file(cfg_path, c.params);
  c.constraints_built = false;
  if (c.finalized) constraints_build(c);
  API_END
}
pnp_status pnp_params_get(pnp_ctx* ctx, double* sys, double* surf, char* meshfile, int meshfile_cap) {
  API_BEGIN(ctx)
  PNP_REQUIRE(c.params.set, PNP_E_ARG, "parameters not set");
  const HostParams& p = c.params;
  const double v[16] = {(double)p.n_surfaces, (double)p.cylindrical, p.l_b, p.c0, p.PI, (double)p.linearSolverIterations,
                        p.newtonReassembleThreshold, p.newtonReduction, p.newtonMinLinearReduction, p.newtonMaxIterations,
                        p.newtonLineSearchMaxIteration, p.tau, (double)p.nSteps, (double)p.outputFreq,
                        (double)p.potentialUpdateFreq, (double)p.verbosity};
  if (sys) std::memcpy(sys, v, sizeof v);
  if (surf)
    for (int i = 0; i < p.n_surfaces; i++)
      for (int k = 0; k < 3; k++) {
        surf[9 * i + 3 * k] = p.surfaces[i].btype[k];
        surf[9 * i + 3 * k + 1] = p.surfaces[i].flux[k];
        surf[9 * i + 3 * k + 2] = p.surfaces[i].dval[k];
      }
  if (meshfile && meshfile_cap > 0) { std::strncpy(meshfile, p.meshfile.c_str(), meshfile_cap - 1); meshfile[meshfile_cap - 1] = 0; }
  API_END
}
pnp_status pnp_constraints_build(pnp_ctx* ctx) { API_BEGIN(ctx) constraints_build(c); API_END }

pnp_status pnp_operator_create(pnp_ctx* ctx, int op, int comp0, int* handle) {
  API_BEGIN(ctx)
  PNP_REQUIRE(op >= PNP_OP_PB && op <= PNP_OP_PNP && comp0 >= 0 && comp0 < 3 && handle, PNP_E_ARG, "bad operator arguments");
  auto o = std::make_unique<Operator>();
  o->op = op; o->comp0 = comp0;
  c.ops.push_back(std::move(o));
  *handle = (int)c.ops.size() - 1;
  API_END
}
pnp_status pnp_operator_set_coefficient(pnp_ctx* ctx, int h, int which, int vec_handle) {
  API_BEGIN(ctx)
  PNP_REQUIRE(which == 0 || which == 1, PNP_E_ARG, "coefficient index must be 0 or 1");
  c.vec(vec_handle);
  (which == 0 ? c.oper(h).aux0 : c.oper(h).aux1) = vec_handle;
  API_END
}
pnp_status pnp_operator_set_valency(pnp_ctx* ctx, int h, double valency) { API_BEGIN(ctx) c.oper(h).valency = valency; API_END }
pnp_status pnp_constraints_get(pnp_ctx* ctx, int h, char* out) {
  API_BEGIN(ctx)
  PNP_REQUIRE(c.constraints_built, PNP_E_ARG, "constraints not built");
  const Operator& op = c.oper(h);
  if (c.degree >= 2) { p2_constraints_get(c, op, out); return PNP_OK; }
  const int F = op_fields(op.op);
  std::vector<unsigned char> m = c.dmask.to_host(c.stream);
  std::vector<int> i2e = c.int2ext.to_host(c.stream);
  for (long v = 0; v < c.nv; v++)
    for (int k = 0; k < F; k++) out[(long)k * c.nv + i2e[v]] = (char)((m[v] >> (F == 3 ? k : op.comp0)) & 1);
  API_END
}
pnp_status pnp_pattern_get(pnp_ctx* ctx, int h, long* nnz, int* rowptr, int* col) {
  API_BEGIN(ctx)
  long n = pattern_export(c, h, rowptr, col);
  if (nnz) *nnz = n;
  API_END
}

pnp_status pnp_vec_create(pnp_ctx* ctx, int fields, int* handle) {
  API_BEGIN(ctx)
  PNP_REQUIRE(c.finalized, PNP_E_ARG, "mesh not finalized");
  PNP_REQUIRE((fields == 1 || fields == 3) && handle, PNP_E_ARG, "fields must be 1 or 3");
  auto v = std::make_unique<Vec>();
  v->fields = fields; v->d.alloc((size_t)fields * c.cols()); v->d.zero(c.stream);
  c.vecs.push_back(std::move(v));
  *handle = (int)c.vecs.size() - 1;
  API_END
}
pnp_status pnp_vec_destroy(pnp_ctx* ctx, int h) {
  API_BEGIN(ctx)
  if (c.vec(h).d.p == c.last_u) { c.last_u = nullptr; c.last_vals = nullptr; }
  c.vecs[h].reset();
  API_END
}
pnp_status pnp_vec_upload(pnp_ctx* ctx, int h, const double* host) { API_BEGIN(ctx) vec_upload(c, c.vec(h), host); API_END }
pnp_status pnp_vec_download(pnp_ctx* ctx, int h, double* host) { API_BEGIN(ctx) vec_download(c, c.vec(h), host); API_END }
pnp_status pnp_vec_set(pnp_ctx* ctx, int h, double value) {
  API_BEGIN(ctx)
  Vec& v = c.vec(h);
  k_fill<<<grid_for((long)v.d.n, 256), 256, 0, c.stream>>>(v.d.p, (long)v.d.n, value);
  PNP_CHECK_LAUNCH(); c.launches++;
  API_END
}
pnp_status pnp_vec_copy(pnp_ctx* ctx, int dst, int src) {
  API_BEGIN(ctx)
  PNP_REQUIRE(c.vec(dst).d.n == c.vec(src).d.n, PNP_E_ARG, "vector sizes differ");
  vec_copy(c, c.vec(src).d.p, c.vec(dst).d.p, (long)c.vec(src).d.n);
  API_END
}
pnp_status pnp_vec_axpy(pnp_ctx* ctx, int y, double a, int x) {
  API_BEGIN(ctx)
  PNP_REQUIRE(c.vec(y).d.n == c.vec(x).d.n, PNP_E_ARG, "vector sizes differ");
  vec_axpy(c, a, c.vec(x).d.p, c.vec(y).d.p, (long)c.vec(x).d.n);
  API_END
}
pnp_status pnp_vec_norm(pnp_ctx* ctx, int x, double* out) {
  API_BEGIN(ctx) *out = vec_norm(c, c.vec(x).d.p, c.rows() * c.vec(x).fields); API_END
}
pnp_status pnp_vec_dot(pnp_ctx* ctx, int x, int y, double* out) {
  API_BEGIN(ctx)
  PNP_REQUIRE(c.vec(y).d.n == c.vec(x).d.n, PNP_E_ARG, "vector sizes differ");
  *out = vec_dot(c, c.vec(x).d.p, c.vec(y).d.p, c.rows() * c.vec(x).fields);
  API_END
}
pnp_status pnp_vec_pack3(pnp_ctx* ctx, int dst3, int phi, int cp, int cm) {
  API_BEGIN(ctx)
  PNP_REQUIRE(c.vec(dst3).fields == 3 && c.vec(phi).fields == 1 && c.vec(cp).fields == 1 && c.vec(cm).fields == 1,
              PNP_E_ARG, "pack3 needs one 3-field and three 1-field vectors");
  if (c.degree >= 2) {
    const int src[3] = {phi, cp, cm};
    for (int k = 0; k < 3; k++) vec_copy(c, c.vec(src[k]).d.p, c.vec(dst3).d.p + k * c.p2_nd, c.p2_nd);
    return PNP_OK;
  }
  k_pack3<<<grid_for(c.nv, 256), 256, 0, c.stream>>>(c.vec(phi).d.p, c.vec(cp).d.p, c.vec(cm).d.p, c.nv, c.vec(dst3).d.p);
  PNP_CHECK_LAUNCH(); c.launches++;
  API_END
}
pnp_status pnp_vec_extract(pnp_ctx* ctx, int src3, int field, int dst1) {
  API_BEGIN(ctx)
  PNP_REQUIRE(c.vec(src3).fields == 3 && c.vec(dst1).fields == 1 && field >= 0 && field < 3, PNP_E_ARG, "bad extract arguments");
  if (c.degree >= 2) { vec_copy(c, c.vec(src3).d.p + field * c.p2_nd, c.vec(dst1).d.p, c.p2_nd); return PNP_OK; }
  k_extract<<<grid_for(c.nv, 256), 256, 0, c.stream>>>(c.vec(src3).d.p, c.nv, field, c.vec(dst1).d.p);
  PNP_CHECK_LAUNCH(); c.launches++;
  API_END
}

pnp_status pnp_matrix_create(pnp_ctx* ctx, int op_handle, int* handle) {
  API_BEGIN(ctx)
  PNP_REQUIRE(c.finalized && handle, PNP_E_ARG, "mesh not finalized");
  auto m = std::make_unique<Matrix>();
  m->op = c.oper(op_handle).op; m->nplanes = op_planes(m->op);
  if (c.degree >= 2) { PNP_REQUIRE(c.constraints_built, PNP_E_ARG, "constraints not built"); p2_matrix_init(c, *m, c.oper(op_handle)); }
  else { m->vals.alloc((size_t)m->nplanes * c.nslots); m->vals.zero(c.stream); }
  c.mats.push_back(std::move(m));
  *handle = (int)c.mats.size() - 1;
  API_END
}
pnp_status pnp_matrix_destroy(pnp_ctx* ctx, int h) {
  API_BEGIN(ctx)
  if (c.mat(h).vals.p == c.last_vals) c.last_vals = nullptr;
  c.mats[h].reset();
  API_END
}
pnp_status pnp_residual(pnp_ctx* ctx, int op, int u, int r) {
  API_BEGIN(ctx)
  assemble_residual(c, c.oper(op), c.vec(u), c.vec(r));
  PNP_CUDA(cudaStreamSynchronize(c.stream));
  API_END
}
pnp_status pnp_jacobian(pnp_ctx* ctx, int op, int u, int A, int mode, double eps) {
  API_BEGIN(ctx)
  assemble_jacobian(c, c.oper(op), c.vec(u), c.mat(A), mode, eps);
  PNP_CUDA(cudaStreamSynchronize(c.stream));
  API_END
}
pnp_status pnp_matrix_values_get(pnp_ctx* ctx, int op, int A, double* val) {
  API_BEGIN(ctx) matrix_export(c, op, c.mat(A), val); API_END
}
pnp_status pnp_spmv(pnp_ctx* ctx, int A, int x, int y) {
  API_BEGIN(ctx)
  const Matrix& M = c.mat(A);
  PNP_REQUIRE(c.vec(x).fields == (M.nplanes == 1 ? 1 : 3) && c.vec(y).fields == c.vec(x).fields && x != y, PNP_E_ARG,
              "spmv operands do not match the matrix");
  spmv(c, M, c.vec(x).d.p, c.vec(y).d.p);
  PNP_CUDA(cudaStreamSynchronize(c.stream));
  API_END
}

pnp_status pnp_solver_create(pnp_ctx* ctx, int kind, int prec, int maxit, int prec_steps, int verbosity, int* handle) {
  API_BEGIN(ctx)
  PNP_REQUIRE((kind == PNP_SOLVER_BCGS || kind == PNP_SOLVER_CG) && prec >= PNP_PREC_NONE && prec <= PNP_PREC_AMG && handle,
              PNP_E_ARG, "bad solver arguments");
  auto s = std::make_unique<Solver>();
  s->kind = kind; s->prec = prec; s->maxit = maxit; s->prec_steps = prec_steps; s->verbosity = verbosity;
  c.solvers.push_back(std::move(s));
  *handle = (int)c.solvers.size() - 1;
  API_END
}
pnp_status pnp_solver_set_option(pnp_ctx* ctx, int s, const char* name, double value) {
  API_BEGIN(ctx)
  PNP_REQUIRE(name, PNP_E_ARG, "null option name");
  c.solver(s).opts[name] = value;
  API_END
}
pnp_status pnp_solver_get(pnp_ctx* ctx, int s, const char* name, double* value) {
  API_BEGIN(ctx)
  PNP_REQUIRE(name && value, PNP_E_ARG, "null argument");
  const std::string n(name);
  if (c.degree >= 2 && (n == "ssor_levels" || n == "ilu0_levels")) *value = c.solver(s).csr_levels;
  else if (n == "ssor_levels") *value = sweep_levels(c.solver(s), false);
  else if (n == "ilu0_levels") *value = sweep_levels(c.solver(s), true);
  else if (n == "amg_graph") *value = amg_graph_state(c.solver(s));
  else PNP_REQUIRE(false, PNP_E_ARG, "unknown solver fact");
  API_END
}
pnp_status pnp_precond_apply(pnp_ctx* ctx, int s, int A, int d, int v) {
  API_BEGIN(ctx)
  precond_apply(c, c.solver(s), c.mat(A), c.vec(d), c.vec(v));
  PNP_CUDA(cudaStreamSynchronize(c.stream));
  API_END
}
pnp_status pnp_solver_apply(pnp_ctx* ctx, int s, int A, int z, int r, double reduction, pnp_lin_result* out) {
  API_BEGIN(ctx)
  LinResult lr = solver_apply(c, c.solver(s), c.mat(A), c.vec(z), c.vec(r), reduction);
  to_lin(lr, out);
  if (lr.status == PNP_E_BREAKDOWN) { c.err = "BiCGSTAB breakdown (rho, omega or h vanished)"; return PNP_E_BREAKDOWN; }
  if (lr.status == PNP_E_NAN) { c.err = "non-finite residual norm in the linear solver"; return PNP_E_NAN; }
  API_END
}

void pnp_newton_opts_default(pnp_newton_opts* o) {
  if (!o) return;
  o->reduction = 1e-8; o->abs_limit = 1e-12; o->min_linear_reduction = 1e-3; o->reassemble_threshold = 0.0;
  o->max_iterations = 40; o->line_search_max_iterations = 10; o->damping = 0.5;
  o->jac_mode = PNP_JAC_FD_FAITHFUL; o->fd_epsilon = 1e-11; o->verbosity = 0;
  o->line_search_strategy = PNP_LS_HACKBUSCH_REUSKEN_ACCEPT_BEST;
}
pnp_status pnp_newton_opts_from_params(pnp_ctx* ctx, pnp_newton_opts* o) {
  API_BEGIN(ctx)
  PNP_REQUIRE(c.params.set && o, PNP_E_ARG, "parameters not set");
  pnp_newton_opts_default(o);
  o->reassemble_threshold = c.params.newtonReassembleThreshold;
  o->reduction = c.params.newtonReduction;
  o->min_linear_reduction = c.params.newtonMinLinearReduction;
  o->max_iterations = (int)c.params.newtonMaxIterations;
  o->line_search_max_iterations = (int)c.params.newtonLineSearchMaxIteration;
  o->verbosity = c.params.verbosity;
  API_END
}
pnp_status pnp_newton_apply(pnp_ctx* ctx, int op, int u, int solver, const pnp_newton_opts* o, pnp_newton_result* res) {
  API_BEGIN(ctx)
  PNP_REQUIRE(o && res, PNP_E_ARG, "null options/result");
  int st = newton_apply(c, c.oper(op), c.vec(u), c.solver(solver), *o, *res);
  if (st != PNP_OK) {
    static const char* msg[] = {"", "Newton did not converge within max_iterations", "linear solver did not converge",
                                "line search failed", "defect is not finite", "BiCGSTAB breakdown"};
    c.err = msg[st <= 5 ? st : 0];
    return st;
  }
  API_END
}
pnp_status pnp_slp_apply(pnp_ctx* ctx, int op, int u, int solver, double reduction, int jac_mode, double eps,
                         pnp_lin_result* out) {
  API_BEGIN(ctx)
  LinResult lr = slp_apply(c, c.oper(op), c.vec(u), c.solver(solver), reduction, jac_mode, eps);
  to_lin(lr, out);
  if (lr.status == PNP_E_BREAKDOWN) { c.err = "BiCGSTAB breakdown (rho, omega or h vanished)"; return PNP_E_BREAKDOWN; }
  if (lr.status == PNP_E_NAN) { c.err = "non-finite residual norm in the linear solver"; return PNP_E_NAN; }
  API_END
}
pnp_status pnp_onestep_apply(pnp_ctx* ctx, int method, int op_space, int op_time, int solver, double time, double dt,
                             int x_old, int dirichlet_values, int x_new, double reduction, int jac_mode, double eps,
                             pnp_lin_result* stage_results) {
  API_BEGIN(ctx)
  (void)time;
  LinResult lr[2];
  const int st = onestep_apply(c, method, c.oper(op_space), c.oper(op_time), c.solver(solver), dt, c.vec(x_old),
                               c.vec(dirichlet_values), c.vec(x_new), reduction, jac_mode, eps, lr);
  if (stage_results) for (int k = 0; k < (method == PNP_TIME_IMPLICIT_EULER ? 1 : 2); k++) to_lin(lr[k], stage_results + k);
  if (st == PNP_E_BREAKDOWN) { c.err = "BiCGSTAB breakdown in a stage solve"; return PNP_E_BREAKDOWN; }
  if (st == PNP_E_NAN) { c.err = "non-finite residual norm in a stage solve"; return PNP_E_NAN; }
  API_END
}
pnp_status pnp_ion_flux(pnp_ctx* ctx, int phi, int cp, int cm, double* ip, double* im) {
  API_BEGIN(ctx)
  PNP_REQUIRE(ip && im, PNP_E_ARG, "null output");
  ion_flux(c, c.vec(phi), c.vec(cp), c.vec(cm), ip, im);
  API_END
}
pnp_status pnp_write_cell_data(pnp_ctx* ctx, int v, const char* filename) {
  API_BEGIN(ctx)
  PNP_REQUIRE(filename, PNP_E_ARG, "null file name");
  write_cell_data(c, c.vec(v), filename);
  API_END
}
pnp_status pnp_write_vtk(pnp_ctx* ctx, const char* name, int n, const int* vec_handles, const char* const* names, int ascii) {
  API_BEGIN(ctx)
  PNP_REQUIRE(name && n >= 0 && (n == 0 || (vec_handles && names)), PNP_E_ARG, "null arguments");
  std::vector<const Vec*> f(n);
  for (int i = 0; i < n; i++) f[i] = &c.vec(vec_handles[i]);
  write_vtk(c, name, n, f.data(), names, ascii);
  API_END
}
pnp_status pnp_matrix_set_csr(pnp_ctx* ctx, int op_handle, int mat_handle, const int* rowptr, const int* col, const double* val) {
  API_BEGIN(ctx) matrix_import(c, op_handle, c.mat(mat_handle), rowptr, col, val); API_END
}
pnp_status pnp_mesh_renumber(pnp_ctx* ctx, const int* new_index) { API_BEGIN(ctx) mesh_renumber(c, new_index); API_END }
pnp_status pnp_mesh_owned(pnp_ctx* ctx, long* n_own) { API_BEGIN(ctx) if (n_own) *n_own = c.n_own; API_END }
pnp_status pnp_interpolate_bcext(pnp_ctx* ctx, int component, int pb_vec, int out_vec) {
  API_BEGIN(ctx)
  PNP_REQUIRE(c.n_own == c.nv, PNP_E_ARG, "interpolate(BCExtension) follows the global element order: run it before partitioning");
  if (c.degree >= 2) p2_interpolate_bcext(c, component, pb_vec >= 0 ? &c.vec(pb_vec) : nullptr, c.vec(out_vec));
  else interpolate_bcext(c, component, pb_vec >= 0 ? &c.vec(pb_vec) : nullptr, c.vec(out_vec));
  API_END
}
pnp_status pnp_space_set_degree(pnp_ctx* ctx, int degree) {
  API_BEGIN(ctx)
  PNP_REQUIRE(degree >= 1 && degree <= 3, PNP_E_ARG, "polynomial degree must be 1, 2 or 3");
  PNP_REQUIRE(!c.finalized, PNP_E_ARG, "set the degree before pnp_mesh_finalize");
  PNP_REQUIRE(degree == 1 || (c.world == 1 && !c.parent), PNP_E_ARG, "quadratic and cubic elements run on one GPU");
  c.degree = degree;
  API_END
}
pnp_status pnp_space_sizes(pnp_ctx* ctx, int* degree, long* n_edges, long* ndof) {
  API_BEGIN(ctx)
  PNP_REQUIRE(c.finalized, PNP_E_ARG, "mesh not finalized");
  if (degree) *degree = c.degree;
  if (c.degree >= 2) p2_sizes(c, n_edges, ndof);
  else { if (n_edges) *n_edges = 0; if (ndof) *ndof = c.nv; }
  API_END
}
pnp_status pnp_space_edges(pnp_ctx* ctx, int* va, int* vb) { API_BEGIN(ctx) p2_edges(c, va, vb); API_END }
pnp_status pnp_space_offsets(pnp_ctx* ctx, long* edge_offset, long* vertex_offset) {
  API_BEGIN(ctx)
  PNP_REQUIRE(c.finalized, PNP_E_ARG, "mesh not finalized");
  if (c.degree >= 2) p2_offsets(c, edge_offset, vertex_offset);
  else { if (edge_offset) *edge_offset = 0; if (vertex_offset) *vertex_offset = 0; }
  API_END
}
pnp_status pnp_operator_set_intorder(pnp_ctx* ctx, int h, int intorder) {
  API_BEGIN(ctx)
  PNP_REQUIRE(intorder == 0 || (intorder == 5 && c.degree >= 2), PNP_E_ARG,
              "quadrature order: 0 (the order the reference's drivers end up with) or, for degree 2 and 3, 5");
  c.oper(h).intorder = intorder;
  API_END
}

}
```

### dune_pnp_b200/csrc/pnp_common.cuh

```cuda
#pragma once
#include <cuda_runtime.h>

#include <cstdint>
#include <cstdio>
#include <map>
#include <memory>
#include <stdexcept>
#include <string>
#include <vector>

#include "../../include/pnp_b200.h"
#include "pnp_setup_algos.cuh"
#include "pnp_star.cuh"

namespace pnp {

struct Error : std::runtime_error {
  int code;
  Error(int c, const std::string& m) : std::runtime_error(m), code(c) {}
};

#define PNP_CUDA(call)                                                                               \
  do {                                                                                               \
    cudaError_t e_ = (call);                                                                         \
    if (e_ != cudaSuccess)                                                                           \
      throw ::pnp::Error(PNP_E_CUDA, std::string(__FILE__) + ":" + std::to_string(__LINE__) + " " +  \
                                         #call + " -> " + cudaGetErrorString(e_));                   \
  } while (0)
#define PNP_CHECK_LAUNCH() PNP_CUDA(cudaGetLastError())
#define PNP_REQUIRE(cond, code, msg)                                                                 \
  do { if (!(cond)) throw ::pnp::Error(code, std::string(msg)); } while (0)

template <class T> struct DBuf {
  T* p = nullptr;
  size_t n = 0;
  DBuf() = default;
  explicit DBuf(size_t n_) { alloc(n_); }
  DBuf(const DBuf&) = delete;
  DBuf& operator=(const DBuf&) = delete;
  DBuf(DBuf&& o) noexcept : p(o.p), n(o.n) { o.p = nullptr; o.n = 0; }
  DBuf& operator=(DBuf&& o) noexcept { if (this != &o) { release(); p = o.p; n = o.n; o.p = nullptr; o.n = 0; } return *this; }
  ~DBuf() { release(); }
  void release() { if (p) cudaFree(p); p = nullptr; n = 0; }
  void alloc(size_t n_) {
    release();
    n = n_;
    if (n) PNP_CUDA(cudaMalloc(&p, n * sizeof(T) + 64));
  }
  void zero(cudaStream_t s) { if (n) PNP_CUDA(cudaMemsetAsync(p, 0, n * sizeof(T), s)); }
  void upload(const T* h, size_t cnt, cudaStream_t s) {
    if (cnt) PNP_CUDA(cudaMemcpyAsync(p, h, cnt * sizeof(T), cudaMemcpyHostToDevice, s));
  }
  void download(T* h, size_t cnt, cudaStream_t s) const {
    if (cnt) PNP_CUDA(cudaMemcpyAsync(h, p, cnt * sizeof(T), cudaMemcpyDeviceToHost, s));
    PNP_CUDA(cudaStreamSynchronize(s));
  }
  std::vector<T> to_host(cudaStream_t s) const { std::vector<T> h(n); download(h.data(), n, s); return h; }
};

struct Tune {
  int tma = 1;
  int tma_stages = 2;
  int tma_lpr = 2;
  long tma_min_rows = -1;
  int graph = 1;
  int fd_warp = 1;
  int jac_compact = 1;
  long p2_chunk = 0;
};
inline Tune& tune() { static Tune t; return t; }

inline int grid_for(long n, int block, int max_blocks = 148 * 32) {
  long g = (n + block - 1) / block;
  if (g < 1) g = 1;
  return (int)(g > max_blocks ? max_blocks : g);
}

struct HostSurface { int btype[3] = {1, 1, 1}; double flux[3] = {0, 0, 0}; double dval[3] = {0, 0, 0}; };
struct HostParams {
  bool set = false;
  int n_surfaces = 0, verbosity = 0, cylindrical = 0;
  double l_b = 1, c0 = 0.06, PI = 3.1415;
  int linearSolverIterations = 50;
  double newtonReassembleThreshold = 0, newtonReduction = 1e-5, newtonMinLinearReduction = 1e-5;
  double newtonMaxIterations = 50, newtonLineSearchMaxIteration = 500, tau = 0.1;
  int nSteps = 100, outputFreq = 1, potentialUpdateFreq = 1;
  std::string meshfile;
  std::vector<HostSurface> surfaces;
};

struct Vec {
  int fields = 1;
  DBuf<double> d;
};
struct Matrix {
  int op = 0;
  int nplanes = 1;
  int comp0 = 0;
  DBuf<double> vals;
  const int* csr_rp = nullptr; const int* csr_col = nullptr; long csr_nnz = 0, csr_n = 0;
  void* csr_pattern = nullptr;
};

struct Operator {
  int op = OP_PB;
  int comp0 = 0;
  double valency = 1.0;
  int aux0 = -1, aux1 = -1;
  int intorder = 0;
};

struct HierLevel {
  long nv = 0, nslots = 0, nE = 0;
  DBuf<int> rp, int2ext, ext2int;
  DBuf<unsigned> adj;
  DBuf<uint64_t> edges;
};

struct Ctx;
struct MgLevelRef {
  Ctx* lc = nullptr;
  DBuf<int> par0, par1;
};

struct Amg;
struct P2Space;
struct SweepPrec;
struct SweepPlan;

struct Solver {
  int kind = PNP_SOLVER_BCGS, prec = PNP_PREC_NONE, maxit = 5000, prec_steps = 1, verbosity = 0;
  std::shared_ptr<Amg> amg;
  std::shared_ptr<SweepPrec> sweep;
  std::map<std::string, double> opts;
  double opt(const char* name, double dflt) const { auto it = opts.find(name); return it == opts.end() ? dflt : it->second; }
  DBuf<double> w[6];
  DBuf<double> dinv;
  DBuf<double> csr_lu; int csr_levels = 0;
  std::shared_ptr<void> pmg;
  void ensure(size_t n) { for (auto& b : w) if (b.n != n) b.alloc(n); if (dinv.n != n) dinv.alloc(n); }
};

struct Ctx {
  int device = 0;
  cudaStream_t stream = nullptr;
  std::string err;
  int sm_count = 148;
  long nv = 0, nT = 0, nB = 0;
  long n_own = 0;
  int degree = 1; long p2_nd = 0;
  std::shared_ptr<P2Space> p2;
  long rows() const { return degree >= 2 ? p2_nd : n_own; }
  long cols() const { return degree >= 2 ? p2_nd : nv; }
  int rank = 0, world = 1;
  void* nccl = nullptr;
  std::vector<int> halo_nbr, halo_send_ptr, halo_recv_ptr;
  std::vector<int> halo_send_ext;
  DBuf<int> halo_send_idx;
  DBuf<double> halo_send_buf;
  DBuf<double> cx, cy;
  DBuf<int> ctri, cba, cbb, cbphys;
  bool finalized = false;
  long nslots = 0;
  DBuf<int> rp;
  DBuf<unsigned> adj;
  DBuf<XY> xy;
  DBuf<unsigned char> dmask;
  DBuf<int> int2ext, ext2int;
  std::vector<BFace> bfaces;
  DBuf<BFace> d_bfaces;
  DBuf<int> d_bv, d_bv_ptr, d_bv_items;
  int n_bv = 0;
  DBuf<double> d_surf;
  DBuf<unsigned char> d_surf_dir;
  HostParams params;
  bool constraints_built = false;
  long launches = 0;
  enum { ACC_SPMV_FINE = 0, ACC_SPMV_COARSE = 1, ACC_ASSEMBLY = 2, ACC_BLAS1 = 3, ACC_TRANSFER = 4, ACC_DENSE = 5, ACC_N = 6 };
  double alg_bytes[ACC_N] = {0, 0, 0, 0, 0, 0};
  void acct(int cls, double bytes) { alg_bytes[cls] += bytes; }
  void absorb(Ctx& child) {
    launches += child.launches; child.launches = 0;
    for (int k = 0; k < ACC_N; k++) { alg_bytes[k] += child.alg_bytes[k]; child.alg_bytes[k] = 0; }
  }
  bool prof = false;
  std::vector<cudaEvent_t> prof_ev;
  std::vector<int> prof_kind;
  size_t prof_used = 0;
  cudaEvent_t tm0 = nullptr, tm1 = nullptr;
  void prof_mark(int kind = 0) {
    if (!prof) return;
    if (prof_used == prof_ev.size()) { cudaEvent_t e; cudaEventCreate(&e); prof_ev.push_back(e); }
    if (prof_used % 2 == 0) { if (prof_kind.size() <= prof_used / 2) prof_kind.resize(prof_used / 2 + 1); prof_kind[prof_used / 2] = kind; }
    cudaEventRecord(prof_ev[prof_used++], stream);
  }
  std::vector<std::unique_ptr<Vec>> vecs;
  std::vector<std::unique_ptr<Matrix>> mats;
  std::vector<std::unique_ptr<Operator>> ops;
  std::vector<std::unique_ptr<Solver>> solvers;
  Vec ws_r, ws_z, ws_prev;
  Matrix ws_A;
  Vec ws_stage[6];
  Matrix ws_B;
  DBuf<double> io_stage;
  bool owns_stream = true;
  std::vector<MgLevelRef> mg;
  DBuf<int> mg_gid; long mg_nglobal = 0; bool mg_aggregated = false;
  Ctx* mg_replica = nullptr;
  long mg_epoch = 0;
  Ctx* parent = nullptr;
  std::vector<Ctx*> children;
  std::vector<void*> owned_children;
  bool owns_comm = false;
  const double* last_u = nullptr; Operator last_op; int last_mode = 0; double last_eps = 1e-11;
  const double* last_vals = nullptr;
  std::vector<HierLevel> hier;
  std::vector<Vec> carry;
  void invalidate_mesh_objects() {
    finalized = false; constraints_built = false; p2.reset(); p2_nd = 0;
    vecs.clear(); mats.clear(); ops.clear(); solvers.clear();
    last_u = nullptr; last_vals = nullptr;
    ws_r.d.release(); ws_z.d.release(); ws_prev.d.release(); ws_A.vals.release(); ws_B.vals.release();
    for (auto& v : ws_stage) v.d.release();
    io_stage.release();
  }
  DBuf<double> red_partial, red_out;
  double* h_red = nullptr;

  StarView star() const { return StarView{rp.p, adj.p, xy.p, dmask.p, (int)n_own}; }
  PhysParams phys(double valency) const {
    PhysParams P; P.PI = params.PI; P.l_b = params.l_b; P.c0 = params.c0; P.valency = valency;
    P.cylindrical = params.cylindrical; return P;
  }
  Vec& vec(int h) { PNP_REQUIRE(h >= 0 && h < (int)vecs.size() && vecs[h], PNP_E_ARG, "bad vector handle"); return *vecs[h]; }
  Matrix& mat(int h) { PNP_REQUIRE(h >= 0 && h < (int)mats.size() && mats[h], PNP_E_ARG, "bad matrix handle"); return *mats[h]; }
  Operator& oper(int h) { PNP_REQUIRE(h >= 0 && h < (int)ops.size() && ops[h], PNP_E_ARG, "bad operator handle"); return *ops[h]; }
  Solver& solver(int h) { PNP_REQUIRE(h >= 0 && h < (int)solvers.size() && solvers[h], PNP_E_ARG, "bad solver handle"); return *solvers[h]; }
};

inline int op_fields(int op) { return op == OP_PNP ? 3 : 1; }
inline int op_planes(int op) { return op == OP_PNP ? 7 : 1; }

void mesh_set(Ctx&, long nv, const double* x, const double* y, long nT, const int* tri, long nB, const int* ba,
              const int* bb, const int* bphys, long n_own);
void mesh_refine(Ctx&, int levels);
void mesh_finalize(Ctx&, bool renumber);
void constraints_build(Ctx&);
void comm_init(Ctx&, int rank, int world, const char* unique_id128);
void comm_unique_id(char* out128);
void comm_destroy(Ctx&);
void comm_bootstrap_file(Ctx&, int rank, int world, const std::string& path);
std::vector<unsigned char> comm_allgatherv(Ctx&, const void* send, long nbytes, std::vector<long>& counts);
void halo_set(Ctx&, int n_nbr, const int* nbr, const int* send_ptr, const int* send_idx, const int* recv_ptr);
void halo_finalize(Ctx&);
void halo_exchange(Ctx&, double* x, int fields);
void allreduce_sum(Ctx&, double* dev, size_t n);
void allreduce_max_u64(Ctx&, unsigned long long* dev, size_t n);
void carry_set(Ctx&, const int* handles, int n);
void carry_get(Ctx&, int i, Vec& out);
void vec_upload(Ctx&, Vec&, const double* host_lex);
void vec_download(Ctx&, const Vec&, double* host_lex);
void vec_from_lex_device(Ctx&, Vec&, const double* d_lex);
void vec_to_lex_device(Ctx&, const Vec&, double* d_lex);
Ctx* ctx_make_owned_child(Ctx& parent);
void ctx_destroy_owned_child(Ctx& parent, Ctx* child);
long pattern_export(Ctx&, int op_handle, int* rowptr, int* col);
void matrix_export(Ctx&, int op_handle, const Matrix&, double* val);
void matrix_import(Ctx&, int op_handle, Matrix&, const int* rowptr, const int* col, const double* val);
void mesh_renumber(Ctx&, const int* new_index);
void read_gmsh_file(const std::string& path, std::vector<double>& x, std::vector<double>& y, std::vector<int>& tri,
                    std::vector<int>& ba, std::vector<int>& bb, std::vector<int>& bphys);
void read_config_file(const std::string& path, HostParams& p);
void interpolate_bcext(Ctx&, int comp, const Vec* pb, Vec& out);
void assemble_residual(Ctx&, const Operator&, Vec& u, Vec& r);
void assemble_jacobian(Ctx&, const Operator&, Vec& u, Matrix& A, int mode, double eps);
void assemble_jacobian_on(Ctx&, const StarView& M, long stride, const Operator&, const double* u, double* vals, int nplanes,
                          int mode, double eps);
void spmv(Ctx&, const Matrix& A, double* x, double* y);
double vec_norm(Ctx&, const double* x, long n);
double vec_dot(Ctx&, const double* x, const double* y, long n);
void vec_axpy(Ctx&, double a, const double* x, double* y, long n);
void vec_copy(Ctx&, const double* x, double* y, long n);
void vec_zero(Ctx&, double* x, long n);
struct LinResult { bool converged = false; int iterations = 0; double reduction = 1, conv_rate = 1; int status = 0; double seconds = 0; };
LinResult solver_apply(Ctx&, Solver&, const Matrix& A, Vec& z, Vec& r, double reduction);
void precond_apply(Ctx&, Solver&, const Matrix& A, Vec& d, Vec& v);
int sweep_levels(const Solver&, bool ilu);
void p2_build(Ctx&);
void p2_constraints(Ctx&);
void p2_matrix_init(Ctx&, Matrix&, const Operator&);
void p2_assemble_residual(Ctx&, const Operator&, Vec& u, Vec& r);
void p2_assemble_jacobian(Ctx&, const Operator&, Vec& u, Matrix& A, int mode, double eps);
void csr_spmv(Ctx&, const Matrix& A, const double* x, double* y);
void csr_diag_inverse(Ctx&, const Matrix& A, double* dinv);
void csr_sweep_setup(Ctx&, Solver&, const Matrix& A, bool ilu);
void csr_ssor_apply(Ctx&, Solver&, const Matrix& A, const double* d, double* y);
void csr_ilu0_apply(Ctx&, Solver&, const Matrix& A, const double* d, double* y);
void pmg_setup(Ctx&, Solver&, const Matrix& A);
void pmg_apply(Ctx&, Solver&, const Matrix& A, const double* d, double* y);
const unsigned char* p2_dirichlet_flags(Ctx&);
void p2_sizes(Ctx&, long* nE, long* nd);
void p2_offsets(Ctx&, long* eoff, long* voff);
void p2_edges(Ctx&, int* eva, int* evb);
void p2_constraints_get(Ctx&, const Operator&, char* out);
long p2_pattern_export(Ctx&, const Operator&, int* rowptr, int* col);
void p2_matrix_import(Ctx&, const Operator&, Matrix&, const int* rowptr, const int* col, const double* val);
void p2_interpolate_bcext(Ctx&, int comp, const Vec* pb, Vec& out);
void p2_ion_flux(Ctx&, const Vec& phi, const Vec& cp, const Vec& cm, double* ip, double* im);
void p2_write_cell_data(Ctx&, const Vec& u, const std::string& filename);
void p2_vertex_values(Ctx&, const Vec& u, double* out);
void ion_flux(Ctx&, const Vec& phi, const Vec& cp, const Vec& cm, double* ip, double* im);
void write_cell_data(Ctx&, const Vec& u, const std::string& filename);
void write_vtk(Ctx&, const std::string& name, int nfields, const Vec* const* fields, const char* const* names, int ascii);

}

struct pnp_ctx { pnp::Ctx c; };
```

### dune_pnp_b200/csrc/pnp_spmv_tma.cuh

```cuda
#pragma once
#include "pnp_spmv.cuh"

namespace pnp {

constexpr int TMA_TR = 128;
constexpr int tma_nw(int lpr) { return TMA_TR * lpr / 32; }
constexpr int tma_producers(int np, int epi, int ndot) { return np + 3 + ((epi != EPI_PLAIN || ndot >= 1) ? 1 : 0); }
constexpr int tma_threads(int np, int epi, int ndot, int lpr) { return (tma_nw(lpr) + tma_producers(np, epi, ndot)) * 32; }
constexpr int TMA_CAP = 960;
constexpr int TMA_MAX_STAGES = 3;
constexpr int TMA_W = 128;

template <int NP> struct TmaLayout {
  static constexpr int F = NP == 1 ? 1 : 3;
  static constexpr int PLANE = (TMA_CAP + 2) * 8;
  static constexpr int COLS = NP * PLANE;
  static constexpr int RP = COLS + (TMA_CAP + 4) * 4;
  static constexpr int B = RP + (TMA_TR + 4) * 4;
  static constexpr int XW = B + (F * TMA_TR + 2) * 8;
  static constexpr int STAGE = XW + (F * (TMA_TR + 2 * TMA_W) + 2) * 8;
  static constexpr int YBUF = TMA_TR * F * 8;
  static constexpr int HEAD = 128;
  static_assert(PLANE % 16 == 0 && COLS % 16 == 0 && RP % 16 == 0 && B % 16 == 0 && XW % 16 == 0 && STAGE % 16 == 0, "bulk copy alignment");
  static constexpr int smem_bytes(int stages) { return HEAD + stages * STAGE + YBUF; }
};

__device__ __forceinline__ unsigned smem_u32(const void* p) { return (unsigned)__cvta_generic_to_shared(p); }
__device__ __forceinline__ void mbar_init(uint64_t* bar, unsigned count) {
  asm volatile("mbarrier.init.shared::cta.b64 [%0], %1;" ::"r"(smem_u32(bar)), "r"(count) : "memory");
}
__device__ __forceinline__ void mbar_expect_tx(uint64_t* bar, unsigned bytes) {
  asm volatile("mbarrier.arrive.expect_tx.shared::cta.b64 _, [%0], %1;" ::"r"(smem_u32(bar)), "r"(bytes) : "memory");
}
__device__ __forceinline__ void mbar_arrive(uint64_t* bar) {
  asm volatile("mbarrier.arrive.shared::cta.b64 _, [%0];" ::"r"(smem_u32(bar)) : "memory");
}
__device__ __forceinline__ void mbar_wait(uint64_t* bar, unsigned parity) {
  unsigned done;
  do {
    asm volatile("{\n .reg .pred p;\n mbarrier.try_wait.parity.shared::cta.b64 p, [%1], %2;\n selp.u32 %0, 1, 0, p;\n}"
                 : "=r"(done) : "r"(smem_u32(bar)), "r"(parity) : "memory");
  } while (!done);
}
__device__ __forceinline__ void bulk_g2s(void* dst, const void* src, unsigned bytes, uint64_t* bar) {
  asm volatile("cp.async.bulk.shared::cluster.global.mbarrier::complete_tx::bytes [%0], [%1], %2, [%3];"
               ::"r"(smem_u32(dst)), "l"(src), "r"(bytes), "r"(smem_u32(bar)) : "memory");
}

template <int NP>
__device__ __forceinline__ void block_inverse_row(const double* dv, int k, double* o) {
  const PnpBlock B = pnp_block<NP>(dv);
  const double a = B.a, b = B.b, c_ = B.c, d = B.d, e = B.e, f = B.f, g = B.g;
  const double det = a * e * g - b * d * g - c_ * e * f;
  const double scale = fabs(a * e * g) + fabs(b * d * g) + fabs(c_ * e * f);
  if (fabs(det) > 1e-12 * scale && scale > 0.0) {
    const double id = 1.0 / det;
    if (k == 0) { o[0] = e * g * id; o[1] = -b * g * id; o[2] = -c_ * e * id; }
    else if (k == 1) { o[0] = -d * g * id; o[1] = (a * g - c_ * f) * id; o[2] = c_ * d * id; }
    else { o[0] = -e * f * id; o[1] = b * f * id; o[2] = (a * e - b * d) * id; }
  } else {
    const double dd = k == 0 ? a : (k == 1 ? e : g);
    const double inv = dd != 0.0 ? 1.0 / dd : 0.0;
    o[0] = k == 0 ? inv : 0.0; o[1] = k == 1 ? inv : 0.0; o[2] = k == 2 ? inv : 0.0;
  }
}

template <int NP, bool STAGED>
__device__ __forceinline__ void slot_product(const StarOpArgs& a, bool ok, int s, const double* sv, const int* vb, const unsigned* sc,
                                             int cbase, const double* sx, int wlo, unsigned wn, double* acc, double* dg) {
  constexpr int F = NP == 1 ? 1 : 3;
  const unsigned c = !ok ? 0u : ((STAGED ? sc[s - cbase] : a.col[s]) & STAR_VMASK);
  const unsigned cw = c - (unsigned)wlo;
  const bool in = cw < wn;
  double x[F], v[NP];
#pragma unroll
  for (int k = 0; k < F; k++) x[k] = !ok ? 0.0 : (in ? sx[F * cw + k] : a.x[(size_t)F * c + k]);
#pragma unroll
  for (int p = 0; p < NP; p++) v[p] = !ok ? 0.0 : (STAGED ? sv[vb[p] + s] : a.vals[(size_t)p * a.stride + s]);
  if (dg) {
#pragma unroll
    for (int p = 0; p < NP; p++) dg[p] = v[p];
  }
  if constexpr (NP == 1) acc[0] += v[0] * x[0];
  else block_mac<NP>(v, x, acc);
}

template <int NP, int EPI, int NDOT, int LPR>
__global__ void __launch_bounds__(tma_threads(NP, EPI, NDOT, LPR), 1) k_star_op_tma(const StarOpArgs a, const int nstages) {
  using L = TmaLayout<NP>;
  constexpr int F = L::F;
  constexpr int TMA_NW = tma_nw(LPR);
  constexpr int RW = 32 / LPR;
  extern __shared__ __align__(128) unsigned char smem[];
  uint64_t* full = reinterpret_cast<uint64_t*>(smem);
  uint64_t* empty = full + TMA_MAX_STAGES;
  unsigned char* stages = smem + L::HEAD;
  double* ybuf = reinterpret_cast<double*>(stages + (size_t)nstages * L::STAGE);
  const int warp = threadIdx.x >> 5, lane = threadIdx.x & 31;
  const int ntiles = (a.nv + TMA_TR - 1) / TMA_TR;
  const int sp = (int)(a.stride & 1);
  if (threadIdx.x == 0) {
    for (int s = 0; s < nstages; s++) { mbar_init(&full[s], tma_producers(NP, EPI, NDOT)); mbar_init(&empty[s], TMA_NW); }
    asm volatile("fence.mbarrier_init.release.cluster;" ::: "memory");
  }
  __syncthreads();
  double dsum[NDOT > 0 ? NDOT : 1];
#pragma unroll
  for (int j = 0; j < (NDOT > 0 ? NDOT : 1); j++) dsum[j] = 0.0;

  if (warp >= TMA_NW) {
    const int role = warp - TMA_NW;
    auto load_batch = [&](int batch, int& lo, int& hi) {
      const long tt = blockIdx.x + (long)(batch * 32 + lane) * gridDim.x;
      lo = 0; hi = 0;
      if (tt < ntiles) { lo = a.rp[tt * TMA_TR]; hi = a.rp[min((int)tt * TMA_TR + TMA_TR, a.nv)]; }
    };
    int cur_lo, cur_hi, nxt_lo, nxt_hi;
    load_batch(0, cur_lo, cur_hi);
    load_batch(1, nxt_lo, nxt_hi);
    int t = blockIdx.x;
    for (int it = 0; t < ntiles; t += gridDim.x, it++) {
      if (it > 0 && (it & 31) == 0) { cur_lo = nxt_lo; cur_hi = nxt_hi; load_batch(it / 32 + 1, nxt_lo, nxt_hi); }
      const int lo = __shfl_sync(0xffffffffu, cur_lo, it & 31), hi = __shfl_sync(0xffffffffu, cur_hi, it & 31);
      if (lane == 0) {
        const int stage = it % nstages;
        const unsigned parity = (unsigned)((it / nstages) & 1);
        mbar_wait(&empty[stage], parity ^ 1u);
        unsigned char* st = stages + (size_t)stage * L::STAGE;
        const int r0 = t * TMA_TR, rows = min(TMA_TR, a.nv - r0);
        const bool staged = hi - lo <= TMA_CAP;
        const void* src = nullptr; void* dst = nullptr; unsigned nb = 0;
        if (role < NP) {
          if (staged) {
            const int o = (lo + role * sp) & 1;
            nb = (unsigned)(((hi - lo + o) + 1) & ~1) * 8u;
            src = a.vals + (size_t)role * a.stride + (lo - o); dst = st + role * L::PLANE;
          }
        } else if (role == NP) {
          if (staged) {
            const int lo_c = lo & ~3;
            nb = (unsigned)(((hi - lo_c) + 3) & ~3) * 4u;
            src = a.col + lo_c; dst = st + L::COLS;
          }
        } else if (role == NP + 1) {
          nb = (unsigned)((rows + 1 + 3) & ~3) * 4u;
          src = a.rp + r0; dst = st + L::RP;
        } else if (role == NP + 2) {
          const int wlo = max(r0 - TMA_W, 0), whi = min(r0 + TMA_TR + TMA_W, a.nv);
          nb = (unsigned)((F * (whi - wlo) + 1) & ~1) * 8u;
          src = a.x + (size_t)F * wlo; dst = st + L::XW;
        } else {
          nb = (unsigned)((F * rows + 1) & ~1) * 8u;
          src = (EPI == EPI_PLAIN ? a.w1 : a.b) + (size_t)F * r0; dst = st + L::B;
        }
        if (nb) { mbar_expect_tx(&full[stage], nb); bulk_g2s(dst, src, nb, &full[stage]); }
        else mbar_arrive(&full[stage]);
      }
      __syncwarp();
    }
  } else {
    const int sub = lane % LPR;
    double* yw = ybuf + warp * RW * F;
    int t = blockIdx.x;
    for (int it = 0; t < ntiles; t += gridDim.x, it++) {
      const int stage = it % nstages;
      const unsigned parity = (unsigned)((it / nstages) & 1);
      mbar_wait(&full[stage], parity);
      const unsigned char* st = stages + (size_t)stage * L::STAGE;
      const double* sv = reinterpret_cast<const double*>(st);
      const unsigned* sc = reinterpret_cast<const unsigned*>(st + L::COLS);
      const int* srp = reinterpret_cast<const int*>(st + L::RP);
      const double* sb = reinterpret_cast<const double*>(st + L::B);
      const double* sx = reinterpret_cast<const double*>(st + L::XW);
      const int r0 = t * TMA_TR, rows = min(TMA_TR, a.nv - r0);
      const int wlo = max(r0 - TMA_W, 0);
      const unsigned wn = (unsigned)(min(r0 + TMA_TR + TMA_W, a.nv) - wlo);
      const double* sxo = sx + (size_t)F * (r0 - wlo);
      const int lo = srp[0], hi = srp[rows];
      const bool staged = hi - lo <= TMA_CAP;
      const int cbase = lo & ~3;
      int vb[NP];
#pragma unroll
      for (int p = 0; p < NP; p++) vb[p] = p * (TMA_CAP + 2) - lo + ((lo + p * sp) & 1);
      const int rl = RW * warp + lane / LPR;
      const bool valid = rl < rows;
      const int b0 = valid ? srp[rl] : hi, e0 = valid ? srp[rl + 1] : hi;
      double acc[F], dg[NP];
#pragma unroll
      for (int k = 0; k < F; k++) acc[k] = 0.0;
#pragma unroll
      for (int p = 0; p < NP; p++) dg[p] = 0.0;
      const int len = e0 - b0;
      const int maxlen = __reduce_max_sync(0xffffffffu, len);
      if (staged) {
        constexpr int MAXS = (8 + LPR - 1) / LPR;
        unsigned cj[MAXS];
        bool okj[MAXS];
        double xj[MAXS][F];
#pragma unroll
        for (int u = 0; u < MAXS; u++) {
          const int j = sub + u * LPR;
          okj[u] = j < len;
          cj[u] = okj[u] ? (sc[b0 + j - cbase] & STAR_VMASK) : 0u;
        }
#pragma unroll
        for (int u = 0; u < MAXS; u++) {
          const unsigned cw = cj[u] - (unsigned)wlo;
          const bool in = cw < wn;
          const bool ldg = okj[u] && !in, lds = okj[u] && in;
#pragma unroll
          for (int k = 0; k < F; k++) {
            double xg = 0.0, xs = 0.0;
            if (ldg) xg = a.x[(size_t)F * cj[u] + k];
            if (lds) xs = sx[F * cw + k];
            xj[u][k] = in ? xs : xg;
          }
        }
#pragma unroll
        for (int u = 0; u < MAXS; u++) {
          const int s = b0 + sub + u * LPR;
          double v[NP];
#pragma unroll
          for (int p = 0; p < NP; p++) v[p] = okj[u] ? sv[vb[p] + s] : 0.0;
          if (EPI == EPI_JACOBI && u == 0) {
#pragma unroll
            for (int p = 0; p < NP; p++) dg[p] = v[p];
          }
          if constexpr (NP == 1) acc[0] += v[0] * xj[u][0];
          else block_mac<NP>(v, xj[u], acc);
        }
        for (int j = sub + MAXS * LPR; j < maxlen; j += LPR)
          slot_product<NP, true>(a, j < len, b0 + j, sv, vb, sc, cbase, sx, wlo, wn, acc, nullptr);
      } else {
        slot_product<NP, false>(a, sub < len, b0 + sub, sv, vb, sc, cbase, sx, wlo, wn, acc, EPI == EPI_JACOBI ? dg : nullptr);
        for (int j = sub + LPR; j < maxlen; j += LPR)
          slot_product<NP, false>(a, j < len, b0 + j, sv, vb, sc, cbase, sx, wlo, wn, acc, nullptr);
      }
      if (LPR > 1) {
#pragma unroll
        for (int k = 0; k < F; k++)
#pragma unroll
          for (int o = LPR / 2; o > 0; o >>= 1) acc[k] += __shfl_xor_sync(0xffffffffu, acc[k], o);
      }
      const bool mine = valid && sub == 0;
      double yv[F];
#pragma unroll
      for (int k = 0; k < F; k++) yv[k] = 0.0;
      if (mine) {
        if (EPI == EPI_PLAIN) {
#pragma unroll
          for (int k = 0; k < F; k++) {
            yv[k] = acc[k];
            if (NDOT >= 1) dsum[0] += acc[k] * sb[F * rl + k];
            if (NDOT >= 2) dsum[NDOT >= 2 ? 1 : 0] += acc[k] * acc[k];
          }
        } else if (EPI == EPI_RESIDUAL) {
#pragma unroll
          for (int k = 0; k < F; k++) yv[k] = sb[F * rl + k] - acc[k];
        } else {
          double r[F], z[F];
#pragma unroll
          for (int k = 0; k < F; k++) r[k] = sb[F * rl + k] - acc[k];
          if constexpr (F == 3) {
#pragma unroll
            for (int k = 0; k < F; k++) {
              double o[3];
              block_inverse_row<NP>(dg, k, o);
              z[k] = o[0] * r[0] + o[1] * r[1] + o[2] * r[2];
            }
          } else z[0] = (dg[0] != 0.0 ? 1.0 / dg[0] : 0.0) * r[0];
#pragma unroll
          for (int k = 0; k < F; k++) yv[k] = sxo[F * rl + k] + a.omega * z[k];
        }
      }
      if (sub == 0) {
#pragma unroll
        for (int k = 0; k < F; k++) yw[F * (lane / LPR) + k] = yv[k];
      }
      __syncwarp();
      {
        const size_t g0 = (size_t)F * (r0 + RW * warp);
        const size_t gend = (size_t)F * a.nv;
#pragma unroll
        for (int i = lane; i < RW * F; i += 32)
          if (g0 + i < gend) a.y[g0 + i] = yw[i];
      }
      __syncwarp();
      if (lane == 0) mbar_arrive(&empty[stage]);
    }
  }
  if (NDOT > 0) {
    __shared__ double sm[NDOT > 0 ? NDOT : 1][TMA_NW];
#pragma unroll
    for (int j = 0; j < (NDOT > 0 ? NDOT : 1); j++) {
      double s = dsum[j];
#pragma unroll
      for (int o = 16; o > 0; o >>= 1) s += __shfl_xor_sync(0xffffffffu, s, o);
      if (lane == 0 && warp < TMA_NW) sm[j][warp] = s;
    }
    __syncthreads();
    if (warp == 0) {
#pragma unroll
      for (int j = 0; j < (NDOT > 0 ? NDOT : 1); j++) {
        double s = lane < TMA_NW ? sm[j][lane] : 0.0;
#pragma unroll
        for (int o = 16; o > 0; o >>= 1) s += __shfl_xor_sync(0xffffffffu, s, o);
        if (lane == 0) a.partial[(long)blockIdx.x * NDOT + j] = s;
      }
    }
  }
}

inline bool star_op_tma_ok(const Ctx& c, const StarOpArgs& a, int epi) {
  const Tune& t = tune();
  if (!t.tma || epi == EPI_CHEBYSHEV) return false;
  if ((long)a.nv < (t.tma_min_rows >= 0 ? t.tma_min_rows : 2l * TMA_TR * c.sm_count)) return false;
  auto al = [](const void* p) { return (reinterpret_cast<uintptr_t>(p) & 15u) == 0; };
  return al(a.rp) && al(a.col) && al(a.vals) && al(a.x) && (!a.b || al(a.b)) && (!a.w1 || al(a.w1));
}

inline int star_op_tma_stages() {
  const int v = tune().tma_stages;
  return v < 2 ? 2 : (v > TMA_MAX_STAGES ? TMA_MAX_STAGES : v);
}

template <int NP, int EPI, int NDOT, int LPR>
inline int launch_star_op_tma_lpr(Ctx& c, const StarOpArgs& a) {
  using L = TmaLayout<NP>;
  const int nstages = star_op_tma_stages();
  const int smem = L::smem_bytes(nstages);
  static unsigned long long configured = 0;
  if (!(configured >> (c.device & 63) & 1ull)) {
    PNP_CUDA(cudaFuncSetAttribute(k_star_op_tma<NP, EPI, NDOT, LPR>, cudaFuncAttributeMaxDynamicSharedMemorySize, L::smem_bytes(TMA_MAX_STAGES)));
    configured |= 1ull << (c.device & 63);
  }
  const int ntiles = (a.nv + TMA_TR - 1) / TMA_TR;
  const int grid = ntiles < c.sm_count ? ntiles : c.sm_count;
  k_star_op_tma<NP, EPI, NDOT, LPR><<<grid, tma_threads(NP, EPI, NDOT, LPR), smem, c.stream>>>(a, nstages);
  PNP_CHECK_LAUNCH(); c.launches++;
  return grid;
}
template <int NP, int EPI, int NDOT>
inline int launch_star_op_tma_inst(Ctx& c, const StarOpArgs& a) {
  return tune().tma_lpr == 2 ? launch_star_op_tma_lpr<NP, EPI, NDOT, 2>(c, a) : launch_star_op_tma_lpr<NP, EPI, NDOT, 1>(c, a);
}

template <int EPI, int NDOT>
inline double star_op_bytes(int nplanes, const StarOpArgs& a) {
  const double F = nplanes == 1 ? 1 : 3, nv = a.nv, ns = a.rp ? (double)a.stride : 0.0;
  double b = (8.0 * nplanes + 4.0) * ns + (4.0 + 16.0 * F) * nv;
  if (EPI != EPI_PLAIN) b += 8.0 * F * nv;
  if (EPI == EPI_PLAIN && NDOT >= 1) b += 8.0 * F * nv;
  if (EPI == EPI_CHEBYSHEV) b += 16.0 * F * nv;
  return b;
}
template <int EPI, int NDOT>
inline int launch_star_op_auto(Ctx& c, int nplanes, const StarOpArgs& a, bool fine = true) {
  c.acct(fine ? Ctx::ACC_SPMV_FINE : Ctx::ACC_SPMV_COARSE, star_op_bytes<EPI, NDOT>(nplanes, a));
  if (EPI != EPI_CHEBYSHEV && star_op_tma_ok(c, a, EPI)) {
    constexpr int E = EPI == EPI_CHEBYSHEV ? EPI_PLAIN : EPI;
    return nplanes == 1 ? launch_star_op_tma_inst<1, E, NDOT>(c, a)
         : nplanes == PNP_COMPACT_PLANES ? launch_star_op_tma_inst<PNP_COMPACT_PLANES, E, NDOT>(c, a)
                                         : launch_star_op_tma_inst<7, E, NDOT>(c, a);
  }
  return launch_star_op<EPI, NDOT>(c, nplanes, a);
}

}
```

Baseline: 446.5 million.

## Fuse consecutive Jacobi sweeps and trailing residual into one TMA kernel

Result: slower. 251.7 million, median of 6 (-43.6%).

```diff
diff --git a/dune_pnp_b200/csrc/pnp_amg.cu b/dune_pnp_b200/csrc/pnp_amg.cu
--- a/dune_pnp_b200/csrc/pnp_amg.cu
+++ b/dune_pnp_b200/csrc/pnp_amg.cu
@@ -36,6 +36,9 @@
   bool redisc = false;
   DBuf<XY> xy_own; DBuf<unsigned char> dmask_own;
   std::shared_ptr<SweepPlan> gs_plan;
+  DBuf<int> fz_ptr, fz_rows; DBuf<double> fz_hx;
+  long fz_slots = 0;
+  bool fuse = false;
 };
 
 }
@@ -69,7 +72,7 @@
   cudaGraphExec_t cg_exec = nullptr;
   bool cg_failed = false;
   int cg_calls = 0;
-  double cg_key[8] = {0, 0, 0, 0, 0, 0, 0, 0};
+  double cg_key[9] = {0, 0, 0, 0, 0, 0, 0, 0, 0};
   std::vector<std::pair<double*, double*>> cg_before, cg_after;
   long cg_launches = 0; double cg_bytes[Ctx::ACC_N] = {0, 0, 0, 0, 0, 0};
   void cg_reset() { if (cg_exec) cudaGraphExecDestroy(cg_exec); cg_exec = nullptr; cg_calls = 0; }
@@ -451,6 +454,44 @@
   if (fine) c.prof_mark(EPI == EPI_RESIDUAL ? 1 : 2);
   launch_star_op_auto<EPI, 0>(c, A.NP, a, fine);
   if (fine) c.prof_mark();
+}
+
+template <int EPI2>
+void level_op2(Ctx& c, const Amg& A, Level& l, const double* x, const double* b, double* x1, double* y) {
+  StarOp2Args f{StarOpArgs{l.rp, l.col, l.vals, l.nslots, l.nv, x, y}, x1, l.fz_ptr.p, l.fz_rows.p, l.fz_hx.p};
+  f.a.b = b; f.a.block = A.F == 3; f.a.omega = A.omega;
+  const bool fine = &l == A.L[0].get();
+  c.acct(fine ? Ctx::ACC_SPMV_FINE : Ctx::ACC_SPMV_COARSE, star_op2_bytes(A.NP, f.a, (long)l.fz_rows.n, l.fz_slots));
+  if (fine) c.prof_mark(2);
+  launch_star_op2<EPI2>(c, A.NP, f);
+  if (fine) c.prof_mark();
+}
+
+void fuse_setup(Ctx& c, const Amg& A, Level& l) {
+  const Tune& t = tune();
+  l.fz_ptr.release(); l.fz_rows.release(); l.fz_hx.release(); l.fz_slots = 0;
+  const long ntiles = (l.nv + TMA_TR - 1) / TMA_TR;
+  const int grid = fuse_grid(c, l.nv);
+  if (A.distributed || c.n_own != c.nv || !(A.NP == 1 || A.NP == PNP_COMPACT_PLANES) || !t.tma || l.nv <= 0) return;
+  if ((long)l.nv < (t.tma_min_rows >= 0 ? t.tma_min_rows : 2l * TMA_TR * c.sm_count) || ntiles < (long)t.mg_fuse_min_tiles * grid) return;
+  std::vector<int> rp((size_t)l.nv + 1);
+  PNP_CUDA(cudaMemcpyAsync(rp.data(), l.rp, rp.size() * sizeof(int), cudaMemcpyDeviceToHost, c.stream));
+  PNP_CUDA(cudaStreamSynchronize(c.stream));
+  std::vector<unsigned> col((size_t)rp[l.nv]);
+  PNP_CUDA(cudaMemcpyAsync(col.data(), l.col, col.size() * sizeof(unsigned), cudaMemcpyDeviceToHost, c.stream));
+  PNP_CUDA(cudaStreamSynchronize(c.stream));
+  const FuseHalo h = fuse_halo_build(rp.data(), col.data(), STAR_VMASK, l.nv, grid);
+  l.fz_ptr.alloc(h.ptr.size()); l.fz_ptr.upload(h.ptr.data(), h.ptr.size(), c.stream);
+  l.fz_rows.alloc(h.rows.size()); l.fz_rows.upload(h.rows.data(), h.rows.size(), c.stream);
+  l.fz_hx.alloc((size_t)A.F * h.rows.size());
+  l.fz_slots = h.slots;
+  PNP_CUDA(cudaStreamSynchronize(c.stream));
+}
+
+bool fuse_applies(const Amg& A, const Level& l, const double* b, const double* x, const double* x2) {
+  auto al = [](const void* p) { return (reinterpret_cast<uintptr_t>(p) & 15u) == 0; };
+  return l.fz_ptr.n > 0 && tune().mg_fuse && tune().tma && A.smoother == 0 && al(l.rp) && al(l.col) && al(l.vals) &&
+         al(b) && al(x) && al(x2) && al(l.r.p);
 }
 
 bool coarsen(Ctx& c, Amg& A, int li) {
@@ -872,13 +913,26 @@
   c.acct(Ctx::ACC_TRANSFER, ((A.F == 3 ? 72.0 : 8.0) + 16.0 * A.F + (dvec ? 8.0 * A.F : 0.0)) * l.nv);
 }
 
-void smooth(Ctx& c, Amg& A, Level& l, int steps, bool zero) {
+void smooth(Ctx& c, Amg& A, Level& l, int steps, bool zero, bool residual = false) {
   const long n = (long)A.F * l.nv;
-  if (steps <= 0) { if (zero) PNP_CUDA(cudaMemsetAsync(l.x.p, 0, n * sizeof(double), c.stream)); return; }
+  if (steps <= 0) {
+    if (zero) PNP_CUDA(cudaMemsetAsync(l.x.p, 0, n * sizeof(double), c.stream));
+    if (residual) level_op<1>(c, A, l, l.x.p, l.b.p, l.r.p);
+    return;
+  }
   if (A.smoother == 0) {
     int s = 0;
     if (zero) { jacobi0(c, A, l, A.omega, nullptr); s = 1; }
+    if (l.fuse && residual && s < steps) {
+      for (; s + 1 < steps; s++) { level_op<2>(c, A, l, l.x.p, l.b.p, l.x2.p); std::swap(l.x.p, l.x2.p); }
+      level_op2<EPI_RESIDUAL>(c, A, l, l.x.p, l.b.p, l.x2.p, l.r.p);
+      std::swap(l.x.p, l.x2.p);
+      return;
+    }
+    if (l.fuse && !residual)
+      for (; s + 1 < steps; s += 2) { level_op2<EPI_JACOBI>(c, A, l, l.x.p, l.b.p, l.r.p, l.x2.p); std::swap(l.x.p, l.x2.p); }
     for (; s < steps; s++) { level_op<2>(c, A, l, l.x.p, l.b.p, l.x2.p); std::swap(l.x.p, l.x2.p); }
+    if (residual) level_op<1>(c, A, l, l.x.p, l.b.p, l.r.p);
     return;
   }
   if (A.smoother == 2) {
@@ -891,6 +945,7 @@
       sweep_gs(c, *l.gs_plan, V, l.vals, l.nslots, l.b.p, l.x.p, -1);
     }
     c.acct(finest ? Ctx::ACC_SPMV_FINE : Ctx::ACC_SPMV_COARSE, 2.0 * steps * ((8.0 * A.NP + 4.0) * (double)l.nslots + 24.0 * n));
+    if (residual) level_op<1>(c, A, l, l.x.p, l.b.p, l.r.p);
     return;
   }
   const double lmx = 1.1 * l.lmax, lmn = l.lmax / A.cheb_ratio;
@@ -905,6 +960,7 @@
     std::swap(l.x.p, l.x2.p);
     rho = rho_new;
   }
+  if (residual) level_op<1>(c, A, l, l.x.p, l.b.p, l.r.p);
 }
 
 void cycle(Ctx& c, Amg& A, int li, int nu, int comp0, bool zero);
@@ -924,8 +980,8 @@
   cudaStreamCaptureStatus cap = cudaStreamCaptureStatusNone;
   PNP_CUDA(cudaStreamIsCapturing(c.stream, &cap));
   if (!tune().graph || A.cg_failed || A.smoother != 0 || cap != cudaStreamCaptureStatusNone) { direct(); return; }
-  const double key[8] = {(double)nu, A.omega, (double)A.gamma, (double)A.wlevels, (double)A.pre_steps, (double)A.post_steps,
-                         (double)A.coarse_sweeps, (double)comp0 + 16.0 * A.dense_n};
+  const double key[9] = {(double)nu, A.omega, (double)A.gamma, (double)A.wlevels, (double)A.pre_steps, (double)A.post_steps,
+                         (double)A.coarse_sweeps, (double)comp0 + 16.0 * A.dense_n, (double)tune().mg_fuse};
   if (A.cg_exec && std::memcmp(key, A.cg_key, sizeof key) != 0) A.cg_reset();
   if (!A.cg_exec) {
     if (A.cg_calls++ < 1) { direct(); return; }
@@ -977,10 +1033,9 @@
     return;
   }
   const int nu_pre = A.pre_steps >= 0 ? A.pre_steps : nu, nu_post = A.post_steps >= 0 ? A.post_steps : nu;
-  smooth(c, A, l, coarsest ? A.coarse_sweeps : nu_pre, zero);
+  smooth(c, A, l, coarsest ? A.coarse_sweeps : nu_pre, zero, !coarsest);
   if (coarsest) return;
   Level& nx = *A.L[li + 1];
-  level_op<1>(c, A, l, l.x.p, l.b.p, l.r.p);
   if (A.distributed) halo_exchange(*l.lc, l.r.p, A.F);
   if (A.F == 1) KL(c, k_restrict<1>, nx.nv, l.agg_ptr.p, l.agg_mem.p, l.par1.p, nx.nv, l.r.p, nx.b.p);
   else KL(c, k_restrict<3>, nx.nv, l.agg_ptr.p, l.agg_mem.p, l.par1.p, nx.nv, l.r.p, nx.b.p);
@@ -1054,6 +1109,7 @@
       level_values(c, A, li, nullptr, comp0);
     }
     for (auto& l : A.L) alloc_work(c, A, *l);
+    for (auto& l : A.L) fuse_setup(c, A, *l);
     if (!A.distributed) {
       Level& l0r = *A.L[0];
       const size_t nall = (size_t)A.F * c.nv;
@@ -1095,7 +1151,9 @@
   if (c.n_own == c.nv) {
     double *keep_b = l0.b.p, *keep_x = l0.x.p, *keep_x2 = l0.x2.p;
     const int pre = A.pre_steps >= 0 ? A.pre_steps : nu, post = A.post_steps >= 0 ? A.post_steps : nu;
-    const int swaps = A.smoother == 2 ? 0 : (pre > 0 ? pre - 1 : 0) + post;
+    for (size_t li = 1; li < A.L.size(); li++) A.L[li]->fuse = fuse_applies(A, *A.L[li], A.L[li]->b.p, A.L[li]->x.p, A.L[li]->x2.p);
+    l0.fuse = fuse_applies(A, l0, d, y, y);
+    const int swaps = A.smoother == 2 ? 0 : (pre > 0 ? pre - 1 : 0) + post - (l0.fuse ? post / 2 : 0);
     struct Restore {
       Level& l; double *b, *x, *x2;
       ~Restore() { l.b.p = b; l.x.p = x; l.x2.p = x2; }
diff --git a/dune_pnp_b200/csrc/pnp_capi.cu b/dune_pnp_b200/csrc/pnp_capi.cu
--- a/dune_pnp_b200/csrc/pnp_capi.cu
+++ b/dune_pnp_b200/csrc/pnp_capi.cu
@@ -224,6 +224,8 @@
   else if (n == "graph") t.graph = value != 0;
   else if (n == "fd_warp") t.fd_warp = value != 0;
   else if (n == "jac_compact") t.jac_compact = value != 0;
+  else if (n == "mg_fuse") t.mg_fuse = value != 0;
+  else if (n == "mg_fuse_min_tiles") t.mg_fuse_min_tiles = (int)value;
   else if (n == "p2_chunk") t.p2_chunk = (long)value;
   else if (n == "tma_min_rows") t.tma_min_rows = (long)value;
   else return PNP_E_ARG;
diff --git a/dune_pnp_b200/csrc/pnp_common.cuh b/dune_pnp_b200/csrc/pnp_common.cuh
--- a/dune_pnp_b200/csrc/pnp_common.cuh
+++ b/dune_pnp_b200/csrc/pnp_common.cuh
@@ -66,6 +66,8 @@
   int graph = 1;
   int fd_warp = 1;
   int jac_compact = 1;
+  int mg_fuse = 1;
+  int mg_fuse_min_tiles = 8;
   long p2_chunk = 0;
 };
 inline Tune& tune() { static Tune t; return t; }
diff --git a/dune_pnp_b200/csrc/pnp_fuse_halo.h b/dune_pnp_b200/csrc/pnp_fuse_halo.h
--- /dev/null
+++ b/dune_pnp_b200/csrc/pnp_fuse_halo.h
@@ -0,0 +1,49 @@
+#pragma once
+#include <algorithm>
+#include <vector>
+
+#ifdef __CUDACC__
+#define PNP_FUSE_HD __host__ __device__ __forceinline__
+#else
+#define PNP_FUSE_HD inline
+#endif
+
+namespace pnp {
+
+constexpr int FUSE_TR = 128;
+
+PNP_FUSE_HD int fuse_chunk_begin(int b, int grid, int ntiles) { return (int)((long long)b * ntiles / grid); }
+
+PNP_FUSE_HD bool fuse_is_halo(unsigned c, int k, int t0, int t1) {
+  const int j = (int)(c / FUSE_TR);
+  return j < t0 || j >= t1 || j > k + 1;
+}
+
+struct FuseHalo {
+  std::vector<int> ptr, rows;
+  long slots = 0;
+};
+inline FuseHalo fuse_halo_build(const int* rp, const unsigned* col, unsigned vmask, int nv, int grid) {
+  FuseHalo h;
+  const int ntiles = (nv + FUSE_TR - 1) / FUSE_TR;
+  h.ptr.assign(1, 0);
+  std::vector<int> mine;
+  for (int b = 0; b < grid; b++) {
+    const int t0 = fuse_chunk_begin(b, grid, ntiles), t1 = fuse_chunk_begin(b + 1, grid, ntiles);
+    mine.clear();
+    const int r1 = std::min(t1 * FUSE_TR, nv);
+    for (int r = t0 * FUSE_TR; r < r1; r++)
+      for (int s = rp[r]; s < rp[r + 1]; s++) {
+        const unsigned c = col[s] & vmask;
+        if ((int)c < nv && fuse_is_halo(c, r / FUSE_TR, t0, t1)) mine.push_back((int)c);
+      }
+    std::sort(mine.begin(), mine.end());
+    mine.erase(std::unique(mine.begin(), mine.end()), mine.end());
+    for (int c : mine) h.slots += rp[c + 1] - rp[c];
+    h.rows.insert(h.rows.end(), mine.begin(), mine.end());
+    h.ptr.push_back((int)h.rows.size());
+  }
+  return h;
+}
+
+}
diff --git a/dune_pnp_b200/csrc/pnp_spmv_tma.cuh b/dune_pnp_b200/csrc/pnp_spmv_tma.cuh
--- a/dune_pnp_b200/csrc/pnp_spmv_tma.cuh
+++ b/dune_pnp_b200/csrc/pnp_spmv_tma.cuh
@@ -1,4 +1,5 @@
 #pragma once
+#include "pnp_fuse_halo.h"
 #include "pnp_spmv.cuh"
 
 namespace pnp {
@@ -65,16 +66,13 @@
   }
 }
 
-template <int NP, bool STAGED>
+template <int NP, bool STAGED, class GX>
 __device__ __forceinline__ void slot_product(const StarOpArgs& a, bool ok, int s, const double* sv, const int* vb, const unsigned* sc,
-                                             int cbase, const double* sx, int wlo, unsigned wn, double* acc, double* dg) {
+                                             int cbase, GX& gx, double* acc, double* dg) {
   constexpr int F = NP == 1 ? 1 : 3;
   const unsigned c = !ok ? 0u : ((STAGED ? sc[s - cbase] : a.col[s]) & STAR_VMASK);
-  const unsigned cw = c - (unsigned)wlo;
-  const bool in = cw < wn;
   double x[F], v[NP];
-#pragma unroll
-  for (int k = 0; k < F; k++) x[k] = !ok ? 0.0 : (in ? sx[F * cw + k] : a.x[(size_t)F * c + k]);
+  gx(c, ok, x);
 #pragma unroll
   for (int p = 0; p < NP; p++) v[p] = !ok ? 0.0 : (STAGED ? sv[vb[p] + s] : a.vals[(size_t)p * a.stride + s]);
   if (dg) {
@@ -84,6 +82,155 @@
   if constexpr (NP == 1) acc[0] += v[0] * x[0];
   else block_mac<NP>(v, x, acc);
 }
+
+template <int NP, int EPI, int NDOT, int LPR>
+__device__ __forceinline__ void tma_produce(const StarOpArgs& a, unsigned char* stages, uint64_t* full, uint64_t* empty, int nstages,
+                                            int first, int step, int tend) {
+  using L = TmaLayout<NP>;
+  constexpr int F = L::F;
+  const int lane = threadIdx.x & 31;
+  const int sp = (int)(a.stride & 1);
+  const int role = (int)(threadIdx.x >> 5) - tma_nw(LPR);
+  auto load_batch = [&](int batch, int& lo, int& hi) {
+    const long tt = first + (long)(batch * 32 + lane) * step;
+    lo = 0; hi = 0;
+    if (tt < tend) { lo = a.rp[tt * TMA_TR]; hi = a.rp[min((int)tt * TMA_TR + TMA_TR, a.nv)]; }
+  };
+  int cur_lo, cur_hi, nxt_lo, nxt_hi;
+  load_batch(0, cur_lo, cur_hi);
+  load_batch(1, nxt_lo, nxt_hi);
+  int t = first;
+  for (int it = 0; t < tend; t += step, it++) {
+    if (it > 0 && (it & 31) == 0) { cur_lo = nxt_lo; cur_hi = nxt_hi; load_batch(it / 32 + 1, nxt_lo, nxt_hi); }
+    const int lo = __shfl_sync(0xffffffffu, cur_lo, it & 31), hi = __shfl_sync(0xffffffffu, cur_hi, it & 31);
+    if (lane == 0) {
+      const int stage = it % nstages;
+      const unsigned parity = (unsigned)((it / nstages) & 1);
+      mbar_wait(&empty[stage], parity ^ 1u);
+      unsigned char* st = stages + (size_t)stage * L::STAGE;
+      const int r0 = t * TMA_TR, rows = min(TMA_TR, a.nv - r0);
+      const bool staged = hi - lo <= TMA_CAP;
+      const void* src = nullptr; void* dst = nullptr; unsigned nb = 0;
+      if (role < NP) {
+        if (staged) {
+          const int o = (lo + role * sp) & 1;
+          nb = (unsigned)(((hi - lo + o) + 1) & ~1) * 8u;
+          src = a.vals + (size_t)role * a.stride + (lo - o); dst = st + role * L::PLANE;
+        }
+      } else if (role == NP) {
+        if (staged) {
+          const int lo_c = lo & ~3;
+          nb = (unsigned)(((hi - lo_c) + 3) & ~3) * 4u;
+          src = a.col + lo_c; dst = st + L::COLS;
+        }
+      } else if (role == NP + 1) {
+        nb = (unsigned)((rows + 1 + 3) & ~3) * 4u;
+        src = a.rp + r0; dst = st + L::RP;
+      } else if (role == NP + 2) {
+        const int wlo = max(r0 - TMA_W, 0), whi = min(r0 + TMA_TR + TMA_W, a.nv);
+        nb = (unsigned)((F * (whi - wlo) + 1) & ~1) * 8u;
+        src = a.x + (size_t)F * wlo; dst = st + L::XW;
+      } else {
+        nb = (unsigned)((F * rows + 1) & ~1) * 8u;
+        src = (EPI == EPI_PLAIN ? a.w1 : a.b) + (size_t)F * r0; dst = st + L::B;
+      }
+      if (nb) { mbar_expect_tx(&full[stage], nb); bulk_g2s(dst, src, nb, &full[stage]); }
+      else mbar_arrive(&full[stage]);
+    }
+    __syncwarp();
+  }
+}
+
+template <int NP, int LPR, bool DIAG, class GX>
+__device__ __forceinline__ void tma_row(const StarOpArgs& a, bool staged, const double* sv, const int* vb, const unsigned* sc,
+                                        int cbase, int b0, int len, GX gx, double* acc, double* dg) {
+  constexpr int F = NP == 1 ? 1 : 3;
+  const int sub = (threadIdx.x & 31) % LPR;
+#pragma unroll
+  for (int k = 0; k < F; k++) acc[k] = 0.0;
+#pragma unroll
+  for (int p = 0; p < NP; p++) dg[p] = 0.0;
+  const int maxlen = __reduce_max_sync(0xffffffffu, len);
+  if (staged) {
+    constexpr int MAXS = (8 + LPR - 1) / LPR;
+    unsigned cj[MAXS];
+    bool okj[MAXS];
+    double xj[MAXS][F];
+#pragma unroll
+    for (int u = 0; u < MAXS; u++) {
+      const int j = sub + u * LPR;
+      okj[u] = j < len;
+      cj[u] = okj[u] ? (sc[b0 + j - cbase] & STAR_VMASK) : 0u;
+    }
+#pragma unroll
+    for (int u = 0; u < MAXS; u++) gx(cj[u], okj[u], xj[u]);
+#pragma unroll
+    for (int u = 0; u < MAXS; u++) {
+      const int s = b0 + sub + u * LPR;
+      double v[NP];
+#pragma unroll
+      for (int p = 0; p < NP; p++) v[p] = okj[u] ? sv[vb[p] + s] : 0.0;
+      if (DIAG && u == 0) {
+#pragma unroll
+        for (int p = 0; p < NP; p++) dg[p] = v[p];
+      }
+      if constexpr (NP == 1) acc[0] += v[0] * xj[u][0];
+      else block_mac<NP>(v, xj[u], acc);
+    }
+    for (int j = sub + MAXS * LPR; j < maxlen; j += LPR)
+      slot_product<NP, true>(a, j < len, b0 + j, sv, vb, sc, cbase, gx, acc, nullptr);
+  } else {
+    slot_product<NP, false>(a, sub < len, b0 + sub, sv, vb, sc, cbase, gx, acc, DIAG ? dg : nullptr);
+    for (int j = sub + LPR; j < maxlen; j += LPR)
+      slot_product<NP, false>(a, j < len, b0 + j, sv, vb, sc, cbase, gx, acc, nullptr);
+  }
+  if (LPR > 1) {
+#pragma unroll
+    for (int k = 0; k < F; k++)
+#pragma unroll
+      for (int o = LPR / 2; o > 0; o >>= 1) acc[k] += __shfl_xor_sync(0xffffffffu, acc[k], o);
+  }
+}
+
+template <int NP, int EPI>
+__device__ __forceinline__ void tma_epilogue(const double* acc, const double* dg, const double* b, const double* x, double omega, double* yv) {
+  constexpr int F = NP == 1 ? 1 : 3;
+  if (EPI == EPI_RESIDUAL) {
+#pragma unroll
+    for (int k = 0; k < F; k++) yv[k] = b[k] - acc[k];
+  } else {
+    double r[F], z[F];
+#pragma unroll
+    for (int k = 0; k < F; k++) r[k] = b[k] - acc[k];
+    if constexpr (F == 3) {
+#pragma unroll
+      for (int k = 0; k < F; k++) {
+        double o[3];
+        block_inverse_row<NP>(dg, k, o);
+        z[k] = o[0] * r[0] + o[1] * r[1] + o[2] * r[2];
+      }
+    } else z[0] = (dg[0] != 0.0 ? 1.0 / dg[0] : 0.0) * r[0];
+#pragma unroll
+    for (int k = 0; k < F; k++) yv[k] = x[k] + omega * z[k];
+  }
+}
+
+template <int F>
+struct WindowGather {
+  const double* x; const double* sx; int wlo; unsigned wn;
+  __device__ __forceinline__ void operator()(unsigned c, bool ok, double* xo) const {
+    const unsigned cw = c - (unsigned)wlo;
+    const bool in = cw < wn;
+    const bool ldg = ok && !in, lds = ok && in;
+#pragma unroll
+    for (int k = 0; k < F; k++) {
+      double xg = 0.0, xs = 0.0;
+      if (ldg) xg = x[(size_t)F * c + k];
+      if (lds) xs = sx[F * cw + k];
+      xo[k] = in ? xs : xg;
+    }
+  }
+};
 
 template <int NP, int EPI, int NDOT, int LPR>
 __global__ void __launch_bounds__(tma_threads(NP, EPI, NDOT, LPR), 1) k_star_op_tma(const StarOpArgs a, const int nstages) {
@@ -109,55 +256,7 @@
   for (int j = 0; j < (NDOT > 0 ? NDOT : 1); j++) dsum[j] = 0.0;
 
   if (warp >= TMA_NW) {
-    const int role = warp - TMA_NW;
-    auto load_batch = [&](int batch, int& lo, int& hi) {
-      const long tt = blockIdx.x + (long)(batch * 32 + lane) * gridDim.x;
-      lo = 0; hi = 0;
-      if (tt < ntiles) { lo = a.rp[tt * TMA_TR]; hi = a.rp[min((int)tt * TMA_TR + TMA_TR, a.nv)]; }
-    };
-    int cur_lo, cur_hi, nxt_lo, nxt_hi;
-    load_batch(0, cur_lo, cur_hi);
-    load_batch(1, nxt_lo, nxt_hi);
-    int t = blockIdx.x;
-    for (int it = 0; t < ntiles; t += gridDim.x, it++) {
-      if (it > 0 && (it & 31) == 0) { cur_lo = nxt_lo; cur_hi = nxt_hi; load_batch(it / 32 + 1, nxt_lo, nxt_hi); }
-      const int lo = __shfl_sync(0xffffffffu, cur_lo, it & 31), hi = __shfl_sync(0xffffffffu, cur_hi, it & 31);
-      if (lane == 0) {
-        const int stage = it % nstages;
-        const unsigned parity = (unsigned)((it / nstages) & 1);
-        mbar_wait(&empty[stage], parity ^ 1u);
-        unsigned char* st = stages + (size_t)stage * L::STAGE;
-        const int r0 = t * TMA_TR, rows = min(TMA_TR, a.nv - r0);
-        const bool staged = hi - lo <= TMA_CAP;
-        const void* src = nullptr; void* dst = nullptr; unsigned nb = 0;
-        if (role < NP) {
-          if (staged) {
-            const int o = (lo + role * sp) & 1;
-            nb = (unsigned)(((hi - lo + o) + 1) & ~1) * 8u;
-            src = a.vals + (size_t)role * a.stride + (lo - o); dst = st + role * L::PLANE;
-          }
-        } else if (role == NP) {
-          if (staged) {
-            const int lo_c = lo & ~3;
-            nb = (unsigned)(((hi - lo_c) + 3) & ~3) * 4u;
-            src = a.col + lo_c; dst = st + L::COLS;
-          }
-        } else if (role == NP + 1) {
-          nb = (unsigned)((rows + 1 + 3) & ~3) * 4u;
-          src = a.rp + r0; dst = st + L::RP;
-        } else if (role == NP + 2) {
-          const int wlo = max(r0 - TMA_W, 0), whi = min(r0 + TMA_TR + TMA_W, a.nv);
-          nb = (unsigned)((F * (whi - wlo) + 1) & ~1) * 8u;
-          src = a.x + (size_t)F * wlo; dst = st + L::XW;
-        } else {
-          nb = (unsigned)((F * rows + 1) & ~1) * 8u;
-          src = (EPI == EPI_PLAIN ? a.w1 : a.b) + (size_t)F * r0; dst = st + L::B;
-        }
-        if (nb) { mbar_expect_tx(&full[stage], nb); bulk_g2s(dst, src, nb, &full[stage]); }
-        else mbar_arrive(&full[stage]);
-      }
-      __syncwarp();
-    }
+    tma_produce<NP, EPI, NDOT, LPR>(a, stages, full, empty, nstages, blockIdx.x, gridDim.x, ntiles);
   } else {
     const int sub = lane % LPR;
     double* yw = ybuf + warp * RW * F;
@@ -186,62 +285,7 @@
       const bool valid = rl < rows;
       const int b0 = valid ? srp[rl] : hi, e0 = valid ? srp[rl + 1] : hi;
       double acc[F], dg[NP];
-#pragma unroll
-      for (int k = 0; k < F; k++) acc[k] = 0.0;
-#pragma unroll
-      for (int p = 0; p < NP; p++) dg[p] = 0.0;
-      const int len = e0 - b0;
-      const int maxlen = __reduce_max_sync(0xffffffffu, len);
-      if (staged) {
-        constexpr int MAXS = (8 + LPR - 1) / LPR;
-        unsigned cj[MAXS];
-        bool okj[MAXS];
-        double xj[MAXS][F];
-#pragma unroll
-        for (int u = 0; u < MAXS; u++) {
-          const int j = sub + u * LPR;
-          okj[u] = j < len;
-          cj[u] = okj[u] ? (sc[b0 + j - cbase] & STAR_VMASK) : 0u;
-        }
-#pragma unroll
-        for (int u = 0; u < MAXS; u++) {
-          const unsigned cw = cj[u] - (unsigned)wlo;
-          const bool in = cw < wn;
-          const bool ldg = okj[u] && !in, lds = okj[u] && in;
-#pragma unroll
-          for (int k = 0; k < F; k++) {
-            double xg = 0.0, xs = 0.0;
-            if (ldg) xg = a.x[(size_t)F * cj[u] + k];
-            if (lds) xs = sx[F * cw + k];
-            xj[u][k] = in ? xs : xg;
-          }
-        }
-#pragma unroll
-        for (int u = 0; u < MAXS; u++) {
-          const int s = b0 + sub + u * LPR;
-          double v[NP];
-#pragma unroll
-          for (int p = 0; p < NP; p++) v[p] = okj[u] ? sv[vb[p] + s] : 0.0;
-          if (EPI == EPI_JACOBI && u == 0) {
-#pragma unroll
-            for (int p = 0; p < NP; p++) dg[p] = v[p];
-          }
-          if constexpr (NP == 1) acc[0] += v[0] * xj[u][0];
-          else block_mac<NP>(v, xj[u], acc);
-        }
-        for (int j = sub + MAXS * LPR; j < maxlen; j += LPR)
-          slot_product<NP, true>(a, j < len, b0 + j, sv, vb, sc, cbase, sx, wlo, wn, acc, nullptr);
-      } else {
-        slot_product<NP, false>(a, sub < len, b0 + sub, sv, vb, sc, cbase, sx, wlo, wn, acc, EPI == EPI_JACOBI ? dg : nullptr);
-        for (int j = sub + LPR; j < maxlen; j += LPR)
-          slot_product<NP, false>(a, j < len, b0 + j, sv, vb, sc, cbase, sx, wlo, wn, acc, nullptr);
-      }
-      if (LPR > 1) {
-#pragma unroll
-        for (int k = 0; k < F; k++)
-#pragma unroll
-          for (int o = LPR / 2; o > 0; o >>= 1) acc[k] += __shfl_xor_sync(0xffffffffu, acc[k], o);
-      }
+      tma_row<NP, LPR, EPI == EPI_JACOBI>(a, staged, sv, vb, sc, cbase, b0, e0 - b0, WindowGather<F>{a.x, sx, wlo, wn}, acc, dg);
       const bool mine = valid && sub == 0;
       double yv[F];
 #pragma unroll
@@ -254,24 +298,7 @@
             if (NDOT >= 1) dsum[0] += acc[k] * sb[F * rl + k];
             if (NDOT >= 2) dsum[NDOT >= 2 ? 1 : 0] += acc[k] * acc[k];
           }
-        } else if (EPI == EPI_RESIDUAL) {
-#pragma unroll
-          for (int k = 0; k < F; k++) yv[k] = sb[F * rl + k] - acc[k];
-        } else {
-          double r[F], z[F];
-#pragma unroll
-          for (int k = 0; k < F; k++) r[k] = sb[F * rl + k] - acc[k];
-          if constexpr (F == 3) {
-#pragma unroll
-            for (int k = 0; k < F; k++) {
-              double o[3];
-              block_inverse_row<NP>(dg, k, o);
-              z[k] = o[0] * r[0] + o[1] * r[1] + o[2] * r[2];
-            }
-          } else z[0] = (dg[0] != 0.0 ? 1.0 / dg[0] : 0.0) * r[0];
-#pragma unroll
-          for (int k = 0; k < F; k++) yv[k] = sxo[F * rl + k] + a.omega * z[k];
-        }
+        } else tma_epilogue<NP, EPI>(acc, dg, sb + F * rl, sxo + F * rl, a.omega, yv);
       }
       if (sub == 0) {
 #pragma unroll
@@ -307,6 +334,156 @@
         for (int o = 16; o > 0; o >>= 1) s += __shfl_xor_sync(0xffffffffu, s, o);
         if (lane == 0) a.partial[(long)blockIdx.x * NDOT + j] = s;
       }
+    }
+  }
+}
+
+struct StarOp2Args {
+  StarOpArgs a;
+  double* x1;
+  const int* hptr; const int* hrows; double* hx;
+};
+constexpr int FUSE_STAGES = 3;
+constexpr int FUSE_RING = 4;
+static_assert(FUSE_TR == TMA_TR, "pnp_fuse_halo.h tiles are the streaming kernels' tiles");
+template <int NP> constexpr int fuse_smem_bytes() { return TmaLayout<NP>::smem_bytes(FUSE_STAGES) + FUSE_RING * TMA_TR * TmaLayout<NP>::F * 8; }
+
+template <int F>
+struct FusedGather {
+  const double* ring; const double* x1; const int* hrows; const double* hx; int h0, h1, t, t0, t1;
+  __device__ __forceinline__ void operator()(unsigned c, bool ok, double* xo) const {
+    if (!ok) {
+#pragma unroll
+      for (int k = 0; k < F; k++) xo[k] = 0.0;
+      return;
+    }
+    const double* q;
+    if (!fuse_is_halo(c, t, t0, t1)) {
+      const int j = (int)(c / TMA_TR);
+      if (j >= t - 1) {
+        q = ring + ((size_t)(j & (FUSE_RING - 1)) * TMA_TR + c % TMA_TR) * F;
+#pragma unroll
+        for (int k = 0; k < F; k++) xo[k] = q[k];
+        return;
+      }
+      q = x1 + (size_t)F * c;
+    } else {
+      int lo = h0, hi = h1;
+      while (lo < hi) { const int m = (lo + hi) >> 1; if ((unsigned)__ldg(hrows + m) < c) lo = m + 1; else hi = m; }
+      q = hx + (size_t)F * lo;
+    }
+#pragma unroll
+    for (int k = 0; k < F; k++) xo[k] = __ldcg(q + k);
+  }
+};
+
+template <int NW>
+__device__ __forceinline__ void consumer_sync() { asm volatile("bar.sync 1, %0;" ::"r"(NW * 32) : "memory"); }
+
+template <int NP, int EPI2, int LPR>
+__global__ void __launch_bounds__(tma_threads(NP, EPI_JACOBI, 0, LPR), 1) k_star_op2_tma(const StarOp2Args f) {
+  const StarOpArgs& a = f.a;
+  using L = TmaLayout<NP>;
+  constexpr int F = L::F;
+  constexpr int TMA_NW = tma_nw(LPR);
+  constexpr int RW = 32 / LPR;
+  extern __shared__ __align__(128) unsigned char smem[];
+  uint64_t* full = reinterpret_cast<uint64_t*>(smem);
+  uint64_t* empty = full + TMA_MAX_STAGES;
+  unsigned char* stages = smem + L::HEAD;
+  double* ybuf = reinterpret_cast<double*>(stages + (size_t)FUSE_STAGES * L::STAGE);
+  double* ring = reinterpret_cast<double*>(stages + (size_t)FUSE_STAGES * L::STAGE + L::YBUF);
+  const int warp = threadIdx.x >> 5, lane = threadIdx.x & 31;
+  const int ntiles = (a.nv + TMA_TR - 1) / TMA_TR;
+  const int t0 = fuse_chunk_begin(blockIdx.x, gridDim.x, ntiles), t1 = fuse_chunk_begin(blockIdx.x + 1, gridDim.x, ntiles);
+  const int sp = (int)(a.stride & 1);
+  if (threadIdx.x == 0) {
+    for (int s = 0; s < FUSE_STAGES; s++) { mbar_init(&full[s], tma_producers(NP, EPI_JACOBI, 0)); mbar_init(&empty[s], TMA_NW); }
+    asm volatile("fence.mbarrier_init.release.cluster;" ::: "memory");
+  }
+  __syncthreads();
+  if (warp >= TMA_NW) {
+    tma_produce<NP, EPI_JACOBI, 0, LPR>(a, stages, full, empty, FUSE_STAGES, t0, 1, t1);
+    return;
+  }
+  const int sub = lane % LPR;
+  double* yw = ybuf + warp * RW * F;
+  const int rl = RW * warp + lane / LPR;
+  const int h0 = f.hptr[blockIdx.x], h1 = f.hptr[blockIdx.x + 1];
+  double acc[F], dg[NP], yv[F];
+  for (int base = h0; base < h1; base += TMA_NW * RW) {
+    const int i = base + rl;
+    const bool v = i < h1;
+    const int row = v ? f.hrows[i] : 0;
+    const int b0 = v ? a.rp[row] : 0, len = v ? a.rp[row + 1] - b0 : 0;
+    tma_row<NP, LPR, true>(a, false, nullptr, nullptr, nullptr, 0, b0, len, WindowGather<F>{a.x, nullptr, 0, 0u}, acc, dg);
+    if (v && sub == 0) {
+      tma_epilogue<NP, EPI_JACOBI>(acc, dg, a.b + (size_t)F * row, a.x + (size_t)F * row, a.omega, yv);
+#pragma unroll
+      for (int k = 0; k < F; k++) f.hx[(size_t)F * i + k] = yv[k];
+    }
+  }
+  consumer_sync<TMA_NW>();
+  struct View { const double* sv; const unsigned* sc; const int* srp; const double* sb; const double* sx; int r0, rows, lo, hi, cbase; int vb[NP]; };
+  auto view = [&](int it, View& w) {
+    const unsigned char* st = stages + (size_t)(it % FUSE_STAGES) * L::STAGE;
+    w.sv = reinterpret_cast<const double*>(st);
+    w.sc = reinterpret_cast<const unsigned*>(st + L::COLS);
+    w.srp = reinterpret_cast<const int*>(st + L::RP);
+    w.sb = reinterpret_cast<const double*>(st + L::B);
+    w.sx = reinterpret_cast<const double*>(st + L::XW);
+    w.r0 = (t0 + it) * TMA_TR; w.rows = min(TMA_TR, a.nv - w.r0);
+    w.lo = w.srp[0]; w.hi = w.srp[w.rows]; w.cbase = w.lo & ~3;
+#pragma unroll
+    for (int p = 0; p < NP; p++) w.vb[p] = p * (TMA_CAP + 2) - w.lo + ((w.lo + p * sp) & 1);
+  };
+  auto store = [&](double* out, int r0) {
+    if (sub == 0) {
+#pragma unroll
+      for (int k = 0; k < F; k++) yw[F * (lane / LPR) + k] = yv[k];
+    }
+    __syncwarp();
+    const size_t g0 = (size_t)F * (r0 + RW * warp), gend = (size_t)F * a.nv;
+#pragma unroll
+    for (int i = lane; i < RW * F; i += 32)
+      if (g0 + i < gend) out[g0 + i] = yw[i];
+    __syncwarp();
+  };
+  const int n = t1 - t0;
+  for (int it = 0; it <= n; it++) {
+    if (it < n) {
+      mbar_wait(&full[it % FUSE_STAGES], (unsigned)((it / FUSE_STAGES) & 1));
+      View w; view(it, w);
+      const int wlo = max(w.r0 - TMA_W, 0);
+      const unsigned wn = (unsigned)(min(w.r0 + TMA_TR + TMA_W, a.nv) - wlo);
+      const double* sxo = w.sx + (size_t)F * (w.r0 - wlo);
+      const bool valid = rl < w.rows;
+      const int b0 = valid ? w.srp[rl] : w.hi, e0 = valid ? w.srp[rl + 1] : w.hi;
+      tma_row<NP, LPR, true>(a, w.hi - w.lo <= TMA_CAP, w.sv, w.vb, w.sc, w.cbase, b0, e0 - b0, WindowGather<F>{a.x, w.sx, wlo, wn}, acc, dg);
+#pragma unroll
+      for (int k = 0; k < F; k++) yv[k] = 0.0;
+      if (valid && sub == 0) {
+        tma_epilogue<NP, EPI_JACOBI>(acc, dg, w.sb + F * rl, sxo + F * rl, a.omega, yv);
+        double* rq = ring + ((size_t)((t0 + it) & (FUSE_RING - 1)) * TMA_TR + rl) * F;
+#pragma unroll
+        for (int k = 0; k < F; k++) rq[k] = yv[k];
+      }
+      store(f.x1, w.r0);
+    }
+    consumer_sync<TMA_NW>();
+    if (it >= 1) {
+      const int t = t0 + it - 1;
+      View w; view(it - 1, w);
+      const bool valid = rl < w.rows;
+      const int b0 = valid ? w.srp[rl] : w.hi, e0 = valid ? w.srp[rl + 1] : w.hi;
+      const double* own = ring + (size_t)(t & (FUSE_RING - 1)) * TMA_TR * F;
+      tma_row<NP, LPR, EPI2 == EPI_JACOBI>(a, w.hi - w.lo <= TMA_CAP, w.sv, w.vb, w.sc, w.cbase, b0, e0 - b0,
+                                            FusedGather<F>{ring, f.x1, f.hrows, f.hx, h0, h1, t, t0, t1}, acc, dg);
+#pragma unroll
+      for (int k = 0; k < F; k++) yv[k] = 0.0;
+      if (valid && sub == 0) tma_epilogue<NP, EPI2>(acc, dg, w.sb + F * rl, own + F * rl, a.omega, yv);
+      store(a.y, w.r0);
+      if (lane == 0) mbar_arrive(&empty[(it - 1) % FUSE_STAGES]);
     }
   }
 }
@@ -345,6 +522,24 @@
   return tune().tma_lpr == 2 ? launch_star_op_tma_lpr<NP, EPI, NDOT, 2>(c, a) : launch_star_op_tma_lpr<NP, EPI, NDOT, 1>(c, a);
 }
 
+inline int fuse_grid(const Ctx& c, int nv) { const int nt = (nv + TMA_TR - 1) / TMA_TR; return nt < c.sm_count ? nt : c.sm_count; }
+template <int NP, int EPI2, int LPR>
+inline void launch_star_op2_tma_lpr(Ctx& c, const StarOp2Args& f) {
+  static unsigned long long configured = 0;
+  if (!(configured >> (c.device & 63) & 1ull)) {
+    PNP_CUDA(cudaFuncSetAttribute(k_star_op2_tma<NP, EPI2, LPR>, cudaFuncAttributeMaxDynamicSharedMemorySize, fuse_smem_bytes<NP>()));
+    configured |= 1ull << (c.device & 63);
+  }
+  k_star_op2_tma<NP, EPI2, LPR><<<fuse_grid(c, f.a.nv), tma_threads(NP, EPI_JACOBI, 0, LPR), fuse_smem_bytes<NP>(), c.stream>>>(f);
+  PNP_CHECK_LAUNCH(); c.launches++;
+}
+template <int EPI2>
+inline void launch_star_op2(Ctx& c, int nplanes, const StarOp2Args& f) {
+  const bool l2 = tune().tma_lpr == 2;
+  if (nplanes == 1) l2 ? launch_star_op2_tma_lpr<1, EPI2, 2>(c, f) : launch_star_op2_tma_lpr<1, EPI2, 1>(c, f);
+  else if (nplanes == PNP_COMPACT_PLANES) l2 ? launch_star_op2_tma_lpr<PNP_COMPACT_PLANES, EPI2, 2>(c, f) : launch_star_op2_tma_lpr<PNP_COMPACT_PLANES, EPI2, 1>(c, f);
+  else throw Error(PNP_E_ARG, "fused smoother pair: 1 or 5 value planes only");
+}
 template <int EPI, int NDOT>
 inline double star_op_bytes(int nplanes, const StarOpArgs& a) {
   const double F = nplanes == 1 ? 1 : 3, nv = a.nv, ns = a.rp ? (double)a.stride : 0.0;
@@ -354,6 +549,11 @@
   if (EPI == EPI_CHEBYSHEV) b += 16.0 * F * nv;
   return b;
 }
+inline double star_op2_bytes(int nplanes, const StarOpArgs& a, long halo_rows, long halo_slots) {
+  const double F = nplanes == 1 ? 1 : 3;
+  return star_op_bytes<EPI_JACOBI, 0>(nplanes, a) + 8.0 * F * a.nv + (8.0 * nplanes + 4.0) * halo_slots + (8.0 + 16.0 * F) * halo_rows;
+}
+
 template <int EPI, int NDOT>
 inline int launch_star_op_auto(Ctx& c, int nplanes, const StarOpArgs& a, bool fine = true) {
   c.acct(fine ? Ctx::ACC_SPMV_FINE : Ctx::ACC_SPMV_COARSE, star_op_bytes<EPI, NDOT>(nplanes, a));
```
